# dmitrii-rudnev/selenite-lite

Hardware: AMD Instinct MI355X
Metric: Msamples/s complex I/Q through full RX chain (whole job) (higher is better)
Workload: dtype f32 in / out / accumulate; FIR multiplicands as exact f16 hi+lo pairs (~22 bits) on the matrix cores

## Files before the change

### include/selenite_rx.h

```cpp
#ifndef SELENITE_RX_H
#define SELENITE_RX_H

#include <stddef.h>
#include <stdint.h>

#ifdef __cplusplus
extern "C" {
#endif

#define SELENITE_RX_ABI_VERSION 2
#define SELENITE_RX_CONFIG_SIZE_V1 112u

#define SELENITE_RX_SUCCESS          0
#define SELENITE_RX_ARGUMENT_ERROR (-1)
#define SELENITE_RX_LENGTH_ERROR   (-2)
#define SELENITE_RX_NANINF         (-4)
#define SELENITE_RX_DEVICE_ERROR   (-7)

#define SELENITE_MODE_LSB 0x00
#define SELENITE_MODE_USB 0x01
#define SELENITE_MODE_CW  0x02
#define SELENITE_MODE_CWR 0x03
#define SELENITE_MODE_AM  0x04
#define SELENITE_MODE_FM  0x08
// ... 59 lines not shown

typedef struct selenite_rx_nr_state_view {
    float *coeffs;
    float *window;
    float *delay;
    float *energy;
    float *x0;
} selenite_rx_nr_state_view;

#define SELENITE_RX_OUT_MONO   0
#define SELENITE_RX_OUT_STEREO 1

typedef struct selenite_rx_out_config {
    uint32_t struct_size;
    uint32_t interp;
    uint32_t ni_taps;
    uint32_t frames;
    const float *coeffs;
} selenite_rx_out_config;

#define SELENITE_RX_WINDOW_HANN            0
#define SELENITE_RX_WINDOW_BLACKMAN_HARRIS 1

typedef struct selenite_rx_spec_config {
    uint32_t struct_size;
    uint32_t fft_len;
    uint32_t stride;
    uint32_t average;
    float alpha;
    const float *window;
} selenite_rx_spec_config;

typedef struct selenite_rx_spec_state_view {
    float *rows;
    float *pending;
    uint64_t *position;
} selenite_rx_spec_state_view;

typedef struct selenite_rx_instance selenite_rx_instance;


int  selenite_rx_init(selenite_rx_instance **S, const selenite_rx_config *cfg);
void selenite_rx_free(selenite_rx_instance *S);

int  selenite_rx_set_mode(selenite_rx_instance *S, uint8_t mode);

int  selenite_rx_status(const selenite_rx_instance *S);
const char *selenite_rx_error_string(const selenite_rx_instance *S);


void selenite_rx_process_f32(selenite_rx_instance *S, const float *pSrcIQ,
                             float *pDstAudio, uint32_t blockSize);

void *selenite_rx_host_alloc(size_t bytes);
void  selenite_rx_host_free(void *hptr);
int   selenite_rx_host_register(void *hptr, size_t bytes);
int   selenite_rx_host_unregister(void *hptr);

void selenite_rx_process_f32_device(selenite_rx_instance *S, const float *dSrcIQ,
                                    float *dDstAudio, uint32_t blockSize);

void selenite_rx_process_q15(selenite_rx_instance *S, const int16_t *pSrcIQ,
                             int16_t *pDstAudio, uint32_t blockSize);
void selenite_rx_process_q15_device(selenite_rx_instance *S, const int16_t *dSrcIQ,
                                    int16_t *dDstAudio, uint32_t blockSize);

void selenite_rx_global_phase1_device(selenite_rx_instance *S, const float *dSrcIQ,
                                      float *dDstAudio, float *dEnv, uint32_t blockSize);
void selenite_rx_global_phase2_device(selenite_rx_instance *S, float *dDstAudio,
                                      const float *dEnv, uint32_t blockSize);

int selenite_rx_global_process_f32_device(selenite_rx_instance *S, const float *dSrcIQ, float *dDstAudio,
                                          uint32_t blockSize, void *rccl_comm);


int selenite_rx_set_guard_ratio(selenite_rx_instance *S, float ratio);
int selenite_rx_guard_stats(selenite_rx_instance *S, uint64_t *guard_blocks, uint64_t *guard_channel_calls,
                            uint64_t *rerun_channel_calls);
int selenite_rx_guard_channels(selenite_rx_instance *S, uint32_t *per_channel);
int selenite_rx_auto_words(selenite_rx_instance *S, uint32_t *per_channel);
int selenite_rx_set_handover_repair(selenite_rx_instance *S, int on);
int selenite_rx_set_auto_launches(selenite_rx_instance *S, int launches);
int selenite_rx_auto_launches_last(const selenite_rx_instance *S);
int selenite_rx_guard_handover(selenite_rx_instance *S, uint64_t *handover_blocks);
int selenite_rx_guard_clear(selenite_rx_instance *S);


int  selenite_rx_set_stream(selenite_rx_instance *S, void *hip_stream);
int  selenite_rx_sync(selenite_rx_instance *S);

int  selenite_rx_get_state(selenite_rx_instance *S, const selenite_rx_state_view *dst);
int  selenite_rx_set_state(selenite_rx_instance *S, const selenite_rx_state_view *src);
int  selenite_rx_reset(selenite_rx_instance *S);


int  selenite_rx_set_nr(selenite_rx_instance *S, const selenite_rx_nr_config *nr);
int  selenite_rx_get_nr_state(selenite_rx_instance *S, const selenite_rx_nr_state_view *dst);
int  selenite_rx_set_nr_state(selenite_rx_instance *S, const selenite_rx_nr_state_view *src);


int      selenite_rx_set_out(selenite_rx_instance *S, const selenite_rx_out_config *out);
uint32_t selenite_rx_out_values(const selenite_rx_instance *S, uint32_t blockSize);
int      selenite_rx_get_out_state(selenite_rx_instance *S, float *interp_state);
int      selenite_rx_set_out_state(selenite_rx_instance *S, const float *interp_state);


int selenite_rx_set_spectrum(selenite_rx_instance *S, const selenite_rx_spec_config *sp);
int selenite_rx_get_spectrum(selenite_rx_instance *S, float *rows, uint64_t *frames);
const float *selenite_rx_spectrum_device(const selenite_rx_instance *S);
int selenite_rx_get_spectrum_state(selenite_rx_instance *S, const selenite_rx_spec_state_view *dst);
int selenite_rx_set_spectrum_state(selenite_rx_instance *S, const selenite_rx_spec_state_view *src);
int selenite_rx_spectrum_twiddles(float *tw, uint32_t fft_len);

void *selenite_rx_device_alloc(size_t bytes);
void  selenite_rx_device_free(void *dptr);
int   selenite_rx_memcpy_h2d(void *dptr, const void *hptr, size_t bytes);
int   selenite_rx_memcpy_d2h(void *hptr, const void *dptr, size_t bytes);
int   selenite_rx_device_count(void);
int   selenite_rx_set_device(int ordinal);


void selenite_rx_synth_iq_host(float *iq, uint32_t first_channel, uint32_t nch,
                               uint64_t first_sample, uint32_t nsamp, uint64_t seed);
int  selenite_rx_synth_iq_device(selenite_rx_instance *S, float *dIQ, uint32_t first_channel,
                                 uint32_t nch, uint64_t first_sample, uint32_t nsamp,
                                 uint64_t seed);

int  selenite_rx_time_process_device(selenite_rx_instance *S, const float *dSrcIQ,
                                     float *dDstAudio, uint32_t blockSize, uint32_t iters,
                                     float *ms_per_call);
int  selenite_rx_time_process_q15_device(selenite_rx_instance *S, const int16_t *dSrcIQ,
                                         int16_t *dDstAudio, uint32_t blockSize, uint32_t iters,
                                         float *ms_per_call);

int  selenite_rx_time_process_each_device(selenite_rx_instance *S, const void *dSrcIQ, void *dDstAudio, uint32_t blockSize,
                                          uint32_t iters, float *ms_each, int q15);
int  selenite_rx_time_streaming_roof_device(selenite_rx_instance *S, const void *dSrcIQ, void *dDstAudio, uint32_t blockSize,
                                            uint32_t iters, float *ms_each, int q15);
int  selenite_rx_time_pattern_roof_device(selenite_rx_instance *S, const void *dSrcIQ, void *dDstAudio, uint32_t blockSize,
                                          uint32_t iters, float *ms_each, int q15, uint32_t work);

#define SELENITE_RX_OPT_FORCE_GENERIC     0
#define SELENITE_RX_OPT_NO_SHARED_LO      1
#define SELENITE_RX_OPT_NO_PERIODIC_LO    2
#define SELENITE_RX_OPT_RERUN_GRID        3
#define SELENITE_RX_OPT_TX_FORCE_GENERIC  4
#define SELENITE_RX_OPT_CW_GRID           5
#define SELENITE_RX_OPT_COUNT             6
int      selenite_rx_set_plan_option(int option, uint32_t value);
uint32_t selenite_rx_get_plan_option(int option);
int  selenite_rx_device_pci_bus_id(int ordinal, char *buf, size_t len);

const char *selenite_rx_kernel_name(const selenite_rx_instance *S);
const char *selenite_rx_nco_path(const selenite_rx_instance *S);

uint64_t selenite_rx_algorithmic_bytes(const selenite_rx_config *cfg, uint32_t blockSize,
                                       uint64_t *read_bytes);


int selenite_rx_design_lowpass(float *coeffs, uint32_t num_taps, double cutoff);
int selenite_rx_design_hilbert(float *hilb, float *delay, uint32_t num_taps);
int selenite_rx_design_bandpass(float *coeffs, uint32_t n_stages, double f0, double q);

int selenite_rx_design_interp(float *coeffs, uint32_t ni_taps, uint32_t interp, double cutoff);

int selenite_rx_design_window(float *w, uint32_t n, int kind);
// ... 8 lines not shown
```

### selenite-lite_amd/csrc/rx_api.hip

```cpp
#include "rx_internal.h"

#include <cmath>
#include <cstddef>
#include <cstdio>
#include <cstdlib>
#include <cstring>
#include <algorithm>
#include <dlfcn.h>
#include <mutex>
#include <thread>

using namespace srx;

static thread_local std::string g_last_error = "";

static int fail(selenite_rx_instance *S, int code, const std::string &msg)
{
    g_last_error = msg;
    if (S) {
        if (S->status == SELENITE_RX_SUCCESS) S->status = code;
        S->err = msg;
    }
    return code;
}
#define HIPCHK(S, call)                                                                     \
    do {                                                                                    \
        hipError_t e_ = (call);                                                             \
        if (e_ != hipSuccess)                                                               \
            return fail((S), SELENITE_RX_DEVICE_ERROR,                                      \
                        std::string(#call) + ": " + hipGetErrorString(e_));                 \
    } while (0)

const float *srx::host_sin_table()
{
    static float table[513];
    static std::once_flag once;
    std::call_once(once, [] {
        for (int n = 0; n <= 512; ++n) {
            const double s = std::sin(2.0 * 3.14159265358979323846 * (double)n / 512.0);
            char buf[32];
            std::snprintf(buf, sizeof buf, "%.8f", s);
            table[n] = std::strtof(buf, nullptr);
        }
    });
    return table;
}

static bool mode_valid(uint8_t m, uint32_t nh_taps)
{
    if (m == SELENITE_MODE_FM) return nh_taps >= 2;
    return m == SELENITE_MODE_LSB || m == SELENITE_MODE_USB || m == SELENITE_MODE_CW ||
           m == SELENITE_MODE_CWR || m == SELENITE_MODE_AM || m == SELENITE_MODE_DIG ||
           m == SELENITE_MODE_PKT;
}

template <typename T>
static hipError_t dev_upload(T **d, const T *h, size_t n)
{
    *d = nullptr;
    if (n == 0) return hipSuccess;
    hipError_t e = hipMalloc((void **)d, n * sizeof(T));
    if (e != hipSuccess) return e;
    return hipMemcpy(*d, h, n * sizeof(T), hipMemcpyHostToDevice);
}
template <typename T>
static hipError_t dev_alloc(T **d, size_t n)
{
    *d = nullptr;
    if (n == 0) return hipSuccess;
    return hipMalloc((void **)d, n * sizeof(T));
}

static void classify_coeffs(selenite_rx_instance *S)
{
    const uint32_t nh = S->cfg.nh_taps;
    S->delay_is_impulse = false;
    S->hilb_odd_only = false;
    if (!nh) return;
    int ones = 0, idx = -1;
    bool rest_zero = true;
    for (uint32_t k = 0; k < nh; ++k) {
        const float v = S->h_delay[k];
        if (v == 1.0f) { ++ones; idx = (int)k; }
        else if (!(v == 0.0f && !std::signbit(v))) rest_zero = false;
    }
    if (ones == 1 && rest_zero) { S->delay_is_impulse = true; S->delay_index = idx; }
    if (nh % 2 == 1) {
        const int c = (int)(nh - 1) / 2;
        bool ok = true;
        for (uint32_t k = 0; k < nh && ok; ++k)
            if ((((int)k - c) & 1) == 0) {
                const float v = S->h_hilb[k];
                if (!(v == 0.0f && !std::signbit(v))) ok = false;
            }
        S->hilb_odd_only = ok;
    }
}

static void free_device(selenite_rx_instance *S)
{
    void *ptrs[] = { S->d_flags, S->d_guard_ch, S->d_rerun_flag, S->d_rerun_list, S->d_hist_ext, S->d_conv_in, S->d_dec_c, S->d_hilb_c, S->d_delay_c, S->d_biq_c, S->d_sintab, S->d_step, S->d_phase,
                     S->d_dec_state, S->d_fir_state, S->d_biq_state, S->d_gain, S->d_scratch, S->d_env, S->d_env_part,
                     S->d_io_in, S->d_io_out, S->d_lo, S->pipe.d_in[0], S->pipe.d_in[1], S->pipe.d_out[0], S->pipe.d_out[1],
                     S->d_nr_coeffs, S->d_nr_window, S->d_nr_delay, S->d_nr_energy, S->d_nr_x0,
                     S->d_out_coeffs, S->d_out_state, S->d_out_audio,
                     S->d_spec_tw, S->d_spec_window, S->d_spec_rows, S->d_spec_pending };
    for (void *p : ptrs)
        if (p) (void)hipFree(p);
    if (S->h_rerun_seen) (void)hipHostFree(S->h_rerun_seen);
    S->h_rerun_seen = nullptr;
    for (int i = 0; i < 2; ++i) {
        if (S->pipe.h_in[i]) (void)hipHostFree(S->pipe.h_in[i]);
        if (S->pipe.h_out[i]) (void)hipHostFree(S->pipe.h_out[i]);
        if (S->pipe.ev_in[i]) (void)hipEventDestroy(S->pipe.ev_in[i]);
        if (S->pipe.ev_done[i]) (void)hipEventDestroy(S->pipe.ev_done[i]);
        if (S->pipe.ev_out[i]) (void)hipEventDestroy(S->pipe.ev_out[i]);
    }
    if (S->pipe.h2d) (void)hipStreamDestroy(S->pipe.h2d);
    if (S->pipe.d2h) (void)hipStreamDestroy(S->pipe.d2h);
    free_fused(S->plan);
    if (S->own_stream) (void)hipStreamDestroy(S->own_stream);
}

static int nr_init_state(selenite_rx_instance *S)
{
    if (S->nr_kind == SELENITE_RX_NR_OFF) return SELENITE_RX_SUCCESS;
    const size_t C = S->cfg.channels, N = S->nr_taps, D = S->nr_delay;
    std::vector<float> w(C * N);
    for (size_t c = 0; c < C; ++c) std::memcpy(&w[c * N], S->h_nr_init.data(), N * sizeof(float));
    HIPCHK(S, hipMemcpyAsync(S->d_nr_coeffs, w.data(), C * N * sizeof(float), hipMemcpyHostToDevice, S->stream));
    HIPCHK(S, hipMemsetAsync(S->d_nr_window, 0, C * (N - 1) * sizeof(float), S->stream));
    HIPCHK(S, hipMemsetAsync(S->d_nr_delay, 0, C * D * sizeof(float), S->stream));
    HIPCHK(S, hipMemsetAsync(S->d_nr_energy, 0, C * sizeof(float), S->stream));
    HIPCHK(S, hipMemsetAsync(S->d_nr_x0, 0, C * sizeof(float), S->stream));
    HIPCHK(S, hipStreamSynchronize(S->stream));
    return SELENITE_RX_SUCCESS;
}

static int out_init_state(selenite_rx_instance *S)
{
    if (!S->out_on || S->out_taps / S->out_interp < 2) return SELENITE_RX_SUCCESS;
    const size_t n = (size_t)S->cfg.channels * (S->out_taps / S->out_interp - 1);
    HIPCHK(S, hipMemsetAsync(S->d_out_state, 0, n * sizeof(float), S->stream));
    HIPCHK(S, hipStreamSynchronize(S->stream));
    return SELENITE_RX_SUCCESS;
}

static int spec_init_state(selenite_rx_instance *S)
{
    if (!S->spec_len) return SELENITE_RX_SUCCESS;
    const size_t n = (size_t)S->cfg.channels * S->spec_len;
    HIPCHK(S, hipMemsetAsync(S->d_spec_rows, 0, n * sizeof(float), S->stream));
    HIPCHK(S, hipMemsetAsync(S->d_spec_pending, 0, 2 * n * sizeof(float), S->stream));
    HIPCHK(S, hipStreamSynchronize(S->stream));
    S->spec_pos = 0;
    return SELENITE_RX_SUCCESS;
}

static int reset_state(selenite_rx_instance *S)
{
    const selenite_rx_config &g = S->cfg;
    const size_t C = g.channels;
    if (g.nd_taps > 1) HIPCHK(S, hipMemsetAsync(S->d_dec_state, 0, C * 2 * (g.nd_taps - 1) * sizeof(float), S->stream));
    if (g.nh_taps > 1) HIPCHK(S, hipMemsetAsync(S->d_fir_state, 0, C * 2 * (g.nh_taps - 1) * sizeof(float), S->stream));
    if (g.n_biquad) HIPCHK(S, hipMemsetAsync(S->d_biq_state, 0, C * 4 * g.n_biquad * sizeof(float), S->stream));
    HIPCHK(S, hipMemsetAsync(S->d_phase, 0, C * sizeof(uint32_t), S->stream));
    HIPCHK(S, hipMemsetAsync(S->d_flags, 0, kFlagWords * sizeof(uint32_t), S->stream));
    HIPCHK(S, hipMemsetAsync(S->d_guard_ch, 0, 3 * C * sizeof(uint32_t), S->stream));
    if (S->d_rerun_flag) HIPCHK(S, hipMemsetAsync(S->d_rerun_flag, 0, C * sizeof(uint32_t), S->stream));
    if (S->d_rerun_list) HIPCHK(S, hipMemsetAsync(S->d_rerun_list, 0, 2 * sizeof(uint32_t), S->stream));
    S->rerun_par = 0;
    std::vector<float> gi(C, g.agc_gain_init);
    HIPCHK(S, hipMemcpyAsync(S->d_gain, gi.data(), C * sizeof(float), hipMemcpyHostToDevice, S->stream));
    HIPCHK(S, hipStreamSynchronize(S->stream));
    S->phase_uniform = true;
    S->phase_host = 0;
    if (int rc = nr_init_state(S)) return rc;
    if (int rc = out_init_state(S)) return rc;
    return spec_init_state(S);
}

static int check_device_flags(selenite_rx_instance *S)
{
    uint32_t f = 0;
// ... 51 lines not shown
            return fail(nullptr, SELENITE_RX_ARGUMENT_ERROR, "selenite_rx_init: q15_rounding is 0 or 1");
    } else {
        return fail(nullptr, SELENITE_RX_ARGUMENT_ERROR, "selenite_rx_init: struct_size matches neither this header's selenite_rx_config nor version 1's");
    }
    own.struct_size = (uint32_t)sizeof(selenite_rx_config);
    const selenite_rx_config *cfg = &own;
    if (cfg->channels == 0 || cfg->block == 0 || cfg->decim == 0)
        return fail(nullptr, SELENITE_RX_ARGUMENT_ERROR, "selenite_rx_init: channels, block, decim must be non-zero");
    if (!mode_valid(cfg->mode, cfg->nh_taps))
        return fail(nullptr, SELENITE_RX_ARGUMENT_ERROR, "selenite_rx_init: unsupported mode (FM needs the FIR pair's delay lines: nh_taps >= 2)");
    if (cfg->arith != SELENITE_ARITH_CMSIS && cfg->arith != SELENITE_ARITH_FMA && cfg->arith != SELENITE_ARITH_SPLIT16 &&
        cfg->arith != SELENITE_ARITH_AUTO)
        return fail(nullptr, SELENITE_RX_ARGUMENT_ERROR, "selenite_rx_init: bad arith");
    if (cfg->nd_taps == 0 && cfg->decim != 1)
        return fail(nullptr, SELENITE_RX_ARGUMENT_ERROR, "selenite_rx_init: decim > 1 needs a decimator (nd_taps)");
    if (cfg->nd_taps && !cfg->dec_coeffs)
        return fail(nullptr, SELENITE_RX_ARGUMENT_ERROR, "selenite_rx_init: dec_coeffs is NULL");
    if (cfg->nh_taps && (!cfg->hilb_coeffs || !cfg->delay_coeffs))
        return fail(nullptr, SELENITE_RX_ARGUMENT_ERROR, "selenite_rx_init: hilb_coeffs / delay_coeffs is NULL");
    if (cfg->n_biquad && !cfg->biquad_coeffs)
        return fail(nullptr, SELENITE_RX_ARGUMENT_ERROR, "selenite_rx_init: biquad_coeffs is NULL");
    if (cfg->nd_taps > 65535 || cfg->nh_taps > 65535 || cfg->decim > 255)
        return fail(nullptr, SELENITE_RX_ARGUMENT_ERROR, "selenite_rx_init: taps > 65535 or decim > 255");
    if (cfg->block % cfg->decim != 0)
        return fail(nullptr, SELENITE_RX_LENGTH_ERROR, "selenite_rx_init: block is not a multiple of decim");

    int ndev = 0;
    if (hipGetDeviceCount(&ndev) != hipSuccess || ndev <= 0)
        return fail(nullptr, SELENITE_RX_DEVICE_ERROR,
                    "selenite_rx_init: no HIP device (this library has no CPU fallback)");

    selenite_rx_instance *S = new selenite_rx_instance();
    S->cfg = *cfg;
    const size_t C = cfg->channels;
    if (cfg->nd_taps) S->h_dec.assign(cfg->dec_coeffs, cfg->dec_coeffs + cfg->nd_taps);
    if (cfg->nh_taps) {
        S->h_hilb.assign(cfg->hilb_coeffs, cfg->hilb_coeffs + cfg->nh_taps);
        S->h_delay.assign(cfg->delay_coeffs, cfg->delay_coeffs + cfg->nh_taps);
    }
    if (cfg->n_biquad) S->h_biq.assign(cfg->biquad_coeffs, cfg->biquad_coeffs + 5 * cfg->n_biquad);
    S->h_step.resize(C);
    for (size_t c = 0; c < C; ++c) S->h_step[c] = cfg->nco_step ? cfg->nco_step[c] : cfg->nco_step_all;
    S->cfg.dec_coeffs = S->h_dec.data(); S->cfg.hilb_coeffs = S->h_hilb.data();
    S->cfg.delay_coeffs = S->h_delay.data(); S->cfg.biquad_coeffs = S->h_biq.data();
    S->cfg.nco_step = S->h_step.data();
    S->steps_uniform = true;
    for (size_t c = 1; c < C; ++c) S->steps_uniform = S->steps_uniform && S->h_step[c] == S->h_step[0];
    S->steps_grid256 = true;
    for (size_t c = 0; c < C; ++c) S->steps_grid256 = S->steps_grid256 && (S->h_step[c] & 0x00FFFFFFu) == 0;
    S->force_generic = plan_option(SELENITE_RX_OPT_FORCE_GENERIC) ? 1 : 0;
    S->no_shared_lo = plan_option(SELENITE_RX_OPT_NO_SHARED_LO) ? 1 : 0;
    S->no_periodic_lo = plan_option(SELENITE_RX_OPT_NO_PERIODIC_LO) ? 1 : 0;

#define INITCHK(call)                                                                        \
    do {                                                                                     \
        hipError_t e_ = (call);                                                              \
        if (e_ != hipSuccess) {                                                              \
            int rc_ = fail(nullptr, SELENITE_RX_DEVICE_ERROR,                                \
                           std::string("selenite_rx_init: " #call ": ") + hipGetErrorString(e_)); \
            free_device(S);                                                                  \
            delete S;                                                                        \
            return rc_;                                                                      \
        }                                                                                    \
    } while (0)

    INITCHK(hipGetDevice(&S->device));
    INITCHK(hipStreamCreateWithFlags(&S->own_stream, hipStreamNonBlocking));
    S->stream = S->own_stream;
    INITCHK(dev_upload(&S->d_dec_c, S->h_dec.data(), S->h_dec.size()));
    INITCHK(dev_upload(&S->d_hilb_c, S->h_hilb.data(), S->h_hilb.size()));
    INITCHK(dev_upload(&S->d_delay_c, S->h_delay.data(), S->h_delay.size()));
    INITCHK(dev_upload(&S->d_biq_c, S->h_biq.data(), S->h_biq.size()));
    INITCHK(dev_upload(&S->d_sintab, host_sin_table(), (size_t)513));
    INITCHK(dev_upload(&S->d_step, S->h_step.data(), C));
    INITCHK(dev_alloc(&S->d_phase, C));
    INITCHK(dev_alloc(&S->d_dec_state, cfg->nd_taps > 1 ? C * 2 * (cfg->nd_taps - 1) : 0));
    INITCHK(dev_alloc(&S->d_fir_state, cfg->nh_taps > 1 ? C * 2 * (cfg->nh_taps - 1) : 0));
    INITCHK(dev_alloc(&S->d_biq_state, C * 4 * cfg->n_biquad));
    INITCHK(dev_alloc(&S->d_gain, C));
    INITCHK(dev_alloc(&S->d_flags, (size_t)kFlagWords));
    INITCHK(dev_alloc(&S->d_guard_ch, 3 * C));
    INITCHK(dev_alloc(&S->d_rerun_flag, cfg->arith == SELENITE_ARITH_AUTO ? C : 0));
    INITCHK(dev_alloc(&S->d_rerun_list, cfg->arith == SELENITE_ARITH_AUTO ? C + 2 : 0));
    if (cfg->arith == SELENITE_ARITH_AUTO) {
        INITCHK(hipHostMalloc(reinterpret_cast<void **>(&S->h_rerun_seen), sizeof(uint32_t), hipHostMallocMapped));
        *S->h_rerun_seen = 0u;
    }
    if (cfg->arith == SELENITE_ARITH_AUTO && cfg->nd_taps >= 2 && cfg->nh_taps >= 2 &&
        split16_template_nd((int)cfg->nd_taps, (int)cfg->decim, (int)cfg->nh_taps) > 0 && !diag_env("SELENITE_RX_NO_HIST_EXT")) {
        S->ext_len = cfg->decim * ((cfg->nh_taps - 1u + 3u) & ~3u);
    }
#undef INITCHK
    classify_coeffs(S);
    if (plan_fused(S->cfg, S->delay_is_impulse, S->delay_index, S->hilb_odd_only, S->plan) != hipSuccess) {
        int rc_ = fail(nullptr, SELENITE_RX_DEVICE_ERROR, "selenite_rx_init: building fused-kernel tables failed");
        free_device(S);
        delete S;
        return rc_;
    }
    int rc = reset_state(S);
    if (rc != SELENITE_RX_SUCCESS) { free_device(S); delete S; return rc; }
    *out = S;
    return SELENITE_RX_SUCCESS;
}

extern "C" void selenite_rx_free(selenite_rx_instance *S)
{
    if (!S) return;
    (void)hipSetDevice(S->device);
    if (S->stream) (void)hipStreamSynchronize(S->stream);
    free_device(S);
    delete S;
}

extern "C" int selenite_rx_set_mode(selenite_rx_instance *S, uint8_t mode)
{
    if (!S) return fail(nullptr, SELENITE_RX_ARGUMENT_ERROR, "selenite_rx_set_mode: S is NULL");
    if (!mode_valid(mode, S->cfg.nh_taps)) {
        g_last_error = "selenite_rx_set_mode: unsupported mode";
        return SELENITE_RX_ARGUMENT_ERROR;
    }
    S->cfg.mode = mode;
    HIPCHK(S, plan_fused(S->cfg, S->delay_is_impulse, S->delay_index, S->hilb_odd_only, S->plan));
    return SELENITE_RX_SUCCESS;
}

extern "C" int selenite_rx_status(const selenite_rx_instance *S) { return S ? S->status : SELENITE_RX_ARGUMENT_ERROR; }
extern "C" const char *selenite_rx_error_string(const selenite_rx_instance *S)
{
    return S ? S->err.c_str() : g_last_error.c_str();
}
extern "C" const char *selenite_rx_kernel_name(const selenite_rx_instance *S)
{
    if (!S) return "";
    if (S->force_generic) return "generic";
    if (S->plan.kind != 0) return S->plan.name;
    if (cw_fused_ok(S->cfg, S->cfg.block)) {
        static thread_local std::string name;
        name = "k_cw_fused<" + std::to_string(S->cfg.n_biquad) + "," + std::to_string(S->cfg.block) + ">";
        return name.c_str();
    }
    return "generic";
}

static bool periodic_lo(const selenite_rx_instance *S)
{
    const selenite_rx_config &g = S->cfg;
    if (!(g.nco_enable && S->steps_uniform && (S->h_step[0] & 0x00FFFFFFu) == 0 && !S->no_periodic_lo)) return false;
    if ((g.arith == SELENITE_ARITH_SPLIT16 || g.arith == SELENITE_ARITH_AUTO) && S->plan.d_btab16 && g.nd_taps)
        return 256u % (g.block / g.decim) == 0 && ssb_split16_periodic_lo(split16_template_nd((int)g.nd_taps, (int)g.decim, (int)g.nh_taps), (int)g.decim, (int)g.nh_taps);
    if (g.arith == SELENITE_ARITH_AUTO) return false;
    return g.arith != SELENITE_ARITH_CMSIS && S->plan.use_mfma && g.nd_taps && g.decim == 4;
}

static bool periodic_lo_per_channel(const selenite_rx_instance *S)
{
    const selenite_rx_config &g = S->cfg;
    if (!(g.nco_enable && S->steps_grid256 && !S->no_periodic_lo && S->plan.kind != 0)) return false;
    if (256u % (g.block / g.decim) != 0) return false;
    const bool split = (g.arith == SELENITE_ARITH_SPLIT16 || g.arith == SELENITE_ARITH_AUTO) && S->plan.d_btab16;
    if (split && g.nd_taps) return ssb_split16_periodic_lo(split16_template_nd((int)g.nd_taps, (int)g.decim, (int)g.nh_taps), (int)g.decim, (int)g.nh_taps);
    if (split) return false;
    const bool exact = g.arith == SELENITE_ARITH_CMSIS || g.arith == SELENITE_ARITH_AUTO;
    return exact || !(S->plan.use_mfma && g.decim == 4);
}

// ... 9 lines not shown
    }
    return periodic_lo(S) ? "shared LO, period 256 samples, held in registers" : "shared LO table per call";
}

extern "C" int selenite_rx_set_stream(selenite_rx_instance *S, void *hip_stream)
{
    if (!S) return SELENITE_RX_ARGUMENT_ERROR;
    hipStream_t next = hip_stream ? (hipStream_t)hip_stream : S->own_stream;
    if (next != S->stream) {
        HIPCHK(S, hipSetDevice(S->device));
        HIPCHK(S, hipStreamSynchronize(S->stream));
        S->stream = next;
    }
    return SELENITE_RX_SUCCESS;
}

extern "C" int selenite_rx_sync(selenite_rx_instance *S)
{
    if (!S) return SELENITE_RX_ARGUMENT_ERROR;
    HIPCHK(S, hipStreamSynchronize(S->stream));
    return check_device_flags(S);
}

extern "C" int selenite_rx_set_guard_ratio(selenite_rx_instance *S, float ratio)
{
    if (!S || !(ratio >= 0.0f)) return SELENITE_RX_ARGUMENT_ERROR;
    S->guard_ratio = ratio;
    return SELENITE_RX_SUCCESS;
}

extern "C" int selenite_rx_guard_stats(selenite_rx_instance *S, uint64_t *guard_blocks, uint64_t *guard_channel_calls,
                                       uint64_t *rerun_channel_calls)
{
    if (!S) return SELENITE_RX_ARGUMENT_ERROR;
    HIPCHK(S, hipSetDevice(S->device));
    HIPCHK(S, hipStreamSynchronize(S->stream));
    const size_t C = S->cfg.channels;
    std::vector<uint32_t> w(2 * C);
    HIPCHK(S, hipMemcpy(w.data(), S->d_guard_ch, 2 * C * sizeof(uint32_t), hipMemcpyDeviceToHost));
    uint64_t blocks = 0, calls = 0;
    for (size_t c = 0; c < C; ++c) { blocks += w[c]; calls += w[C + c]; }
    if (guard_blocks) *guard_blocks = blocks;
    if (guard_channel_calls) *guard_channel_calls = calls;
    if (rerun_channel_calls) *rerun_channel_calls = S->cfg.arith == SELENITE_ARITH_AUTO ? calls : 0;
    return SELENITE_RX_SUCCESS;
}

extern "C" int selenite_rx_guard_channels(selenite_rx_instance *S, uint32_t *per_channel)
{
    if (!S || !per_channel) return SELENITE_RX_ARGUMENT_ERROR;
    HIPCHK(S, hipSetDevice(S->device));
    HIPCHK(S, hipStreamSynchronize(S->stream));
    HIPCHK(S, hipMemcpy(per_channel, S->d_guard_ch, (size_t)S->cfg.channels * sizeof(uint32_t), hipMemcpyDeviceToHost));
    return SELENITE_RX_SUCCESS;
}

extern "C" int selenite_rx_auto_words(selenite_rx_instance *S, uint32_t *per_channel)
{
    if (!S || !per_channel) return SELENITE_RX_ARGUMENT_ERROR;
    HIPCHK(S, hipSetDevice(S->device));
    HIPCHK(S, hipStreamSynchronize(S->stream));
    if (!S->d_rerun_flag) { std::memset(per_channel, 0, (size_t)S->cfg.channels * sizeof(uint32_t)); return SELENITE_RX_SUCCESS; }
    HIPCHK(S, hipMemcpy(per_channel, S->d_rerun_flag, (size_t)S->cfg.channels * sizeof(uint32_t), hipMemcpyDeviceToHost));
    return SELENITE_RX_SUCCESS;
}

extern "C" int selenite_rx_guard_clear(selenite_rx_instance *S)
{
    if (!S) return SELENITE_RX_ARGUMENT_ERROR;
    HIPCHK(S, hipSetDevice(S->device));
    HIPCHK(S, hipMemsetAsync(S->d_guard_ch, 0, 3 * (size_t)S->cfg.channels * sizeof(uint32_t), S->stream));
    return SELENITE_RX_SUCCESS;
}

extern "C" int selenite_rx_set_auto_launches(selenite_rx_instance *S, int launches)
{
    if (!S || !(launches == 1 || launches == 3)) return SELENITE_RX_ARGUMENT_ERROR;
    S->auto_launches = launches;
    return SELENITE_RX_SUCCESS;
}

extern "C" int selenite_rx_auto_launches_last(const selenite_rx_instance *S)
{
    return S ? (int)S->auto_form_last : 0;
}

extern "C" int selenite_rx_set_handover_repair(selenite_rx_instance *S, int on)
{
    if (!S) return SELENITE_RX_ARGUMENT_ERROR;
    S->handover_repair = on != 0;
    if (!S->handover_repair && S->d_hist_ext) {
        HIPCHK(S, hipSetDevice(S->device));
        HIPCHK(S, hipStreamSynchronize(S->stream));
        const size_t C = S->cfg.channels;
        std::vector<uint32_t> w(C);
        HIPCHK(S, hipMemcpy(w.data(), S->d_rerun_flag, C * sizeof(uint32_t), hipMemcpyDeviceToHost));
        for (size_t c = 0; c < C; ++c)
            if (((w[c] >> kProvShift) & kProvMask) == kProvSplitExt)
                w[c] = (w[c] & ~((kProvMask << kProvShift) | kExtQ15)) | (kProvSplit << kProvShift);
        HIPCHK(S, hipMemcpy(S->d_rerun_flag, w.data(), C * sizeof(uint32_t), hipMemcpyHostToDevice));
        HIPCHK(S, hipFree(S->d_hist_ext));
        S->d_hist_ext = nullptr;
    }
    return SELENITE_RX_SUCCESS;
}

static int ensure_hist_ext(selenite_rx_instance *S)
{
    if (S->d_hist_ext || !S->ext_len || !S->handover_repair || !S->d_rerun_flag) return SELENITE_RX_SUCCESS;
    const size_t n = 2 * (size_t)S->cfg.channels * S->ext_len;
    HIPCHK(S, hipMalloc((void **)&S->d_hist_ext, n * sizeof(float2)));
    HIPCHK(S, hipMemsetAsync(S->d_hist_ext, 0, n * sizeof(float2), S->stream));
    return SELENITE_RX_SUCCESS;
}

extern "C" int selenite_rx_guard_handover(selenite_rx_instance *S, uint64_t *handover_blocks)
{
    if (!S || !handover_blocks) return SELENITE_RX_ARGUMENT_ERROR;
    HIPCHK(S, hipSetDevice(S->device));
    HIPCHK(S, hipStreamSynchronize(S->stream));
    const size_t C = S->cfg.channels;
    std::vector<uint32_t> w(C);
    HIPCHK(S, hipMemcpy(w.data(), S->d_guard_ch + 2 * C, C * sizeof(uint32_t), hipMemcpyDeviceToHost));
    uint64_t n = 0;
    for (size_t c = 0; c < C; ++c) n += w[c];
    *handover_blocks = n;
    return SELENITE_RX_SUCCESS;
}

extern "C" int selenite_rx_reset(selenite_rx_instance *S)
{
    if (!S) return SELENITE_RX_ARGUMENT_ERROR;
    return reset_state(S);
}

static void nr_release(selenite_rx_instance *S)
{
    float **bufs[] = { &S->d_nr_coeffs, &S->d_nr_window, &S->d_nr_delay, &S->d_nr_energy, &S->d_nr_x0 };
    for (float **b : bufs) {
        if (*b) (void)hipFree(*b);
        *b = nullptr;
    }
    S->nr_kind = SELENITE_RX_NR_OFF;
    S->nr_taps = S->nr_delay = 0;
    S->nr_mu = 0.0f;
    S->h_nr_init.clear();
}

extern "C" int selenite_rx_set_nr(selenite_rx_instance *S, const selenite_rx_nr_config *nr)
{
    if (!S) return fail(nullptr, SELENITE_RX_ARGUMENT_ERROR, "selenite_rx_set_nr: S is NULL");
    if (nr && nr->struct_size != sizeof(selenite_rx_nr_config)) {
        g_last_error = "selenite_rx_set_nr: struct_size is not sizeof(selenite_rx_nr_config)";
        return SELENITE_RX_ARGUMENT_ERROR;
    }
    if (nr && nr->kind != SELENITE_RX_NR_OFF) {
        const uint32_t N = nr->num_taps;
        const char *bad = nullptr;
        if (nr->kind != SELENITE_RX_NR_DENOISE && nr->kind != SELENITE_RX_NR_NOTCH) bad = "kind is not a SELENITE_RX_NR_* value";
        else if (N != 8 && N != 16 && N != 32 && N != 64) bad = "num_taps is not 8, 16, 32 or 64";
        else if (nr->delay < 1 || nr->delay > 64) bad = "delay is not 1 .. 64";
        else if (!(nr->mu > 0.0f && nr->mu < 2.0f)) bad = "mu is not finite in (0, 2)";
        else if (nr->coeffs_init)
            for (uint32_t k = 0; k < N && !bad; ++k)
                if (!std::isfinite(nr->coeffs_init[k])) bad = "coeffs_init holds a non-finite weight";
        if (bad) {
            g_last_error = std::string("selenite_rx_set_nr: ") + bad;
// ... 259 lines not shown
    q.coeffs = S->d_nr_coeffs; q.window = S->d_nr_window; q.delay_line = S->d_nr_delay; q.energy = S->d_nr_energy; q.x0 = S->d_nr_x0;
    q.flags = p.flags;
    if (S->sub_count) {
        const size_t c0 = S->sub_first;
        q.coeffs += c0 * S->nr_taps; q.window += c0 * (S->nr_taps - 1); q.delay_line += c0 * S->nr_delay;
        q.energy += c0; q.x0 += c0;
    }
    return q;
}

static int ensure(selenite_rx_instance *S, void **buf, size_t *cap, size_t need)
{
    if (*cap >= need) return SELENITE_RX_SUCCESS;
    if (*buf) { HIPCHK(S, hipStreamSynchronize(S->stream)); HIPCHK(S, hipFree(*buf)); *buf = nullptr; *cap = 0; }
    HIPCHK(S, hipMalloc(buf, need));
    *cap = need;
    return SELENITE_RX_SUCCESS;
}

static bool block_size_ok(selenite_rx_instance *S, uint32_t block_size, const char *who)
{
    if (block_size == 0 || block_size % S->cfg.block != 0) {
        fail(S, SELENITE_RX_LENGTH_ERROR, std::string(who) + ": blockSize is not a non-zero multiple of cfg.block");
        return false;
    }
    return true;
}

enum Phase { kAll, kPhase1, kPhase2 };

static int run_part(selenite_rx_instance *S, const void *src, bool src_q15, void *dst, bool dst_q15,
                    uint32_t block_size, Phase phase, float *ext_env, uint32_t in_stride, uint32_t out_stride)
{
    const selenite_rx_config &g = S->cfg;
    HIPCHK(S, hipSetDevice(S->device));
    if (phase != kPhase2 && S->plan.kind != 0 && S->plan.d_btab16 && !S->force_generic)
        if (int rc = ensure_hist_ext(S)) return rc;
    RxParams p = make_params(S, block_size);
    p.in_stride = in_stride; p.out_stride = out_stride;
    if (front_generic_lds_bytes(p) > 64 * 1024 && (S->force_generic || S->plan.kind == 0))
        return fail(S, SELENITE_RX_LENGTH_ERROR, "filter lengths exceed the LDS budget of the generic kernel");
    const int arith = (int)g.arith;
    const int garith = arith == SELENITE_ARITH_AUTO ? SELENITE_ARITH_CMSIS : arith;
    const bool global = g.agc_enable && g.agc_global;
    const bool cw = mode_is_cw(g.mode) && g.n_biquad;
    const bool nr = phase != kPhase2 && S->nr_kind != SELENITE_RX_NR_OFF;
    hipStream_t st = S->stream;

    const uint32_t phase_now = S->phase_host;
    auto commit_phase = [&]() { if (phase != kPhase2 && g.nco_enable) S->phase_host = phase_now + block_size * S->h_step[0]; };

    const bool fusable = phase != kPhase2 && !S->force_generic;
    const bool ssb_fused = fusable && S->plan.kind != 0;
    const bool cw_fused = fusable && cw_fused_ok(g, block_size) && cw_strides_ok(p.in_stride, p.out_stride);
    if ((global || nr) && src_q15 && (ssb_fused || cw_fused)) {
        const size_t nval = ((size_t)(p.channels - 1) * p.in_stride + block_size) * 2;
        if (nval % 8 == 0) {
            int rc = ensure(S, (void **)&S->d_conv_in, &S->conv_in_bytes, nval * sizeof(float));
            if (rc) return rc;
            HIPCHK(S, launch_q15_to_f32(static_cast<const int16_t *>(src), S->d_conv_in, nval, S->stream));
            src = S->d_conv_in;
            src_q15 = false;
        }
    }
    float *audio = (float *)dst;
    if (dst_q15 && (global || nr || !(ssb_fused || cw_fused))) {
        const size_t need = (size_t)g.channels * p.out_stride * sizeof(float);
        int rc = ensure(S, (void **)&S->d_scratch, &S->scratch_bytes, need);
        if (rc) return rc;
        audio = S->d_scratch;
    }
    if (phase != kPhase2 && S->d_rerun_flag && !ssb_fused) {
        uint32_t *words = S->d_rerun_flag + (S->sub_count ? S->sub_first : 0u);
        if (p.hist_ext) {
            RxParams ph = p;
            ph.chan_flags = words;
            HIPCHK(S, launch_hist_exact(ph, true, st));
        }
        HIPCHK(S, hipMemsetAsync(words, 0, p.channels * sizeof(uint32_t), st));
    }
    bool env_emitted = false;
    if (ssb_fused || cw_fused) {
        RxParams pf = p;
        if (g.nco_enable && S->steps_uniform && S->phase_uniform && !S->no_shared_lo) {
            const uint32_t lo_n = block_size < 256u ? 256u : block_size;
            if (!(S->lo_valid && S->lo_phase == phase_now && S->lo_step == S->h_step[0] && S->lo_n >= lo_n)) {
                S->lo_valid = false;
                int rc = ensure(S, (void **)&S->d_lo, &S->lo_bytes, (size_t)lo_n * sizeof(float2));
                if (rc) return rc;
                HIPCHK(S, launch_lo_table(S->d_lo, S->d_sintab, phase_now, S->h_step[0], lo_n, st));
                S->lo_valid = true; S->lo_phase = phase_now; S->lo_step = S->h_step[0]; S->lo_n = lo_n;
            }
            pf.nco = 2;
            pf.lo = S->d_lo;
            pf.lo_period = periodic_lo(S) ? 256u : 0u;
        } else if (ssb_fused && g.nco_enable && periodic_lo_per_channel(S)) {
            pf.lo_period = 256u;
        }
        if (arith == SELENITE_ARITH_AUTO && ssb_fused) {
            pf.rerun_flag = S->d_rerun_flag + (S->sub_count ? S->sub_first : 0u);
            pf.chan_list = S->d_rerun_list + 2;
            pf.chan_count = S->d_rerun_list;
            pf.rerun_par_host = &S->rerun_par;
            pf.rerun_seen = S->h_rerun_seen;
            pf.auto_inline = S->auto_launches == 1 ? 1u : 0u;
            pf.form_host = &S->auto_form_last;
        }
        void *fdst = dst;
        bool fq15 = dst_q15;
        if (global || nr) {
            pf.agc = 0; fdst = audio; fq15 = false;
            pf.out_cached = 1;
            if (!nr && ssb_fused && (arith == SELENITE_ARITH_SPLIT16 || arith == SELENITE_ARITH_AUTO) && S->plan.d_btab16 && g.nd_taps && g.decim == 4 && (g.block / g.decim) / 4 == 16 &&
                (block_size / g.decim) % 256 == 0 && g.nco_enable && g.mode != SELENITE_MODE_AM && g.mode != SELENITE_MODE_FM) {
                const size_t need = sizeof(float) * env_fold_scratch_floats(p.channels, block_size / g.block);
                int rc = ensure(S, (void **)&S->d_env_part, &S->env_part_cap, need);
                if (rc) return rc;
                pf.env_part = S->d_env_part;
                env_emitted = true;
            }
        }
        if (ssb_fused) HIPCHK(S, launch_fused(S->plan, pf, arith, src, src_q15, fdst, fq15, S->delay_index, st));
        else HIPCHK(S, launch_cw_fused(pf, src, src_q15, fdst, fq15, st));
        commit_phase();
        if (!global && !nr) return SELENITE_RX_SUCCESS;
    }

    if (phase != kPhase2 && !(ssb_fused || cw_fused)) {
        HIPCHK(S, launch_front_generic(p, garith, src, src_q15, audio, st));
        commit_phase();
        if (cw) HIPCHK(S, launch_biquad_generic(p, garith, audio, st));
    }
    if (nr) HIPCHK(S, launch_nlms(make_nr_params(S, p), S->nr_taps, audio, st));
    if (global) {
        float *env = ext_env;
        if (!env) {
            const size_t need = sizeof(float) * (block_size / g.block);
            int rc = ensure(S, (void **)&S->d_env, &S->env_cap, need);
            if (rc) return rc;
            env = S->d_env;
        }
        if (phase != kPhase2) {
            if (env_emitted) {
                HIPCHK(S, launch_env_fold(S->d_env_part, env, p.channels, block_size / g.block, st));
            } else {
                const size_t need = sizeof(float) * env_global_rows(p) * (block_size / g.block);
                int rc = ensure(S, (void **)&S->d_env_part, &S->env_part_cap, need);
                if (rc) return rc;
                HIPCHK(S, launch_env_global(p, audio, S->d_env_part, env, st));
            }
        }
        if (phase != kPhase1) HIPCHK(S, launch_agc_apply_global(p, garith, audio, env, dst, dst_q15, st));
    } else if (g.agc_enable || dst_q15) {
        HIPCHK(S, launch_agc_generic(p, garith, audio, dst, dst_q15, st));
    }
    return SELENITE_RX_SUCCESS;
}

static int run_chain_core(selenite_rx_instance *S, const void *src, bool src_q15, void *dst, bool dst_q15,
                          uint32_t block_size, Phase phase, float *ext_env)
{
    const selenite_rx_config &g = S->cfg;
    const uint32_t nout = block_size / g.decim;
    const bool global = g.agc_enable && g.agc_global;
    if (phase == kAll && !global && !S->force_generic && S->plan.kind != 0 && fused_tail_split(S->plan, g, block_size)) {
        const uint32_t unit = split16_pass_out(g.block, g.decim) * g.decim, bs1 = block_size / unit * unit;
        {
            int rc = run_part(S, src, src_q15, dst, dst_q15, bs1, kAll, nullptr, block_size, nout);
            if (rc) return rc;
            const size_t ein = src_q15 ? sizeof(int16_t) : sizeof(float), eout = dst_q15 ? sizeof(int16_t) : sizeof(float);
            const char *src2 = static_cast<const char *>(src) + (size_t)bs1 * 2 * ein;
            char *dst2 = static_cast<char *>(dst) + (size_t)(bs1 / g.decim) * eout;
            return run_part(S, src2, src_q15, dst2, dst_q15, block_size - bs1, kAll, nullptr, block_size, nout);
        }
    }
    return run_part(S, src, src_q15, dst, dst_q15, block_size, phase, ext_env, block_size, nout);
}

static int out_audio(selenite_rx_instance *S, uint32_t block_size, float **audio)
{
    const size_t nch = S->sub_count ? S->sub_count : S->cfg.channels;
    int rc = ensure(S, (void **)&S->d_out_audio, &S->out_audio_bytes, nch * (block_size / S->cfg.decim) * sizeof(float));
    *audio = S->d_out_audio;
    return rc;
}
static int out_finish(selenite_rx_instance *S, const float *audio, void *dst, bool dst_q15, uint32_t block_size)
{
    OutParams q{};
// ... 524 lines not shown
```

### selenite-lite_amd/csrc/rx_fused.hip

```cpp
#include "rx_fused_kernels.h"

#include <cmath>
#include <cstdio>
#include <cstdlib>

#pragma clang fp contract(off)

namespace srx {

template <int ND, int M, int NH>
struct GeoM {
    using G = Geo<ND, M, NH>;
    static constexpr int HS = G::HQ4 * M;
    static constexpr int XN = HS + G::T;
    static constexpr int XROWS = XN / 64;
    static constexpr int XLEN = 66 * XROWS;
    static constexpr int KTOT = ND + 4 * 15 + 1;
    static constexpr int KS = (KTOT + 3) / 4;
    static constexpr int oTab = 0;
    static constexpr int oX = 516;
    static constexpr int oD = oX + 2 * XLEN;
    static constexpr int total = oD + 2 * G::DLEN;
    __host__ __device__ static constexpr int phys(int f) { return f + 2 * (f >> 6); }
};
// ... 340 lines not shown
        if (NH > 0) {
            const int nds = split16_template_nd(ndr, M, NH);
            constexpr int MT = M == 8 ? 4 : M;
#define X(ND_, M_, NH_) if (nds == ND_ && MT == M_ && NH == NH_) return build_split16_table<ND_, M_, NH_>(g, plan);
            SRX_SPLIT16_SHAPES(X)
#undef X
        }
        return hipSuccess;
    }
    if constexpr (ND == 0 && M == 1 && NH > 0) {
        using GH = GeoH<NH>;
        float cmax = 0.0f;
        for (int k = 0; k < NH; ++k) cmax = std::fmax(cmax, std::fabs(g.hilb_coeffs[k]));
        int ex = 0;
        if (cmax > 0.0f) std::frexp(cmax, &ex);
        const int SC = 15 - ex;
        std::vector<_Float16> b16((size_t)GH::KS * 2 * 64 * 8, (_Float16)0.0f);
        for (int kk = 0; kk < GH::KS; ++kk)
            for (int l = 0; l < 64; ++l)
                for (int j = 0; j < 8; ++j) {
                    const int idx = 32 * kk + 8 * (l >> 4) + j - (l & 15);
                    float cv = 0.0f;
                    if (idx >= 0 && idx < NH) cv = std::ldexp(g.hilb_coeffs[idx], SC);
                    const _Float16 hi = (_Float16)cv;
                    const _Float16 lo = (_Float16)(cv - (float)hi);
                    b16[(((size_t)2 * kk + 0) * 64 + l) * 8 + j] = hi;
                    b16[(((size_t)2 * kk + 1) * 64 + l) * 8 + j] = lo;
                }
        hipError_t e = hipMalloc(&plan.d_btab16, b16.size() * sizeof(_Float16));
        if (e != hipSuccess) return e;
        e = hipMemcpy(plan.d_btab16, b16.data(), b16.size() * sizeof(_Float16), hipMemcpyHostToDevice);
        if (e != hipSuccess) return e;
        plan.split_sc = SC;
    }
    return hipSuccess;
}


template <int ND, int M, int NH, typename TIn, typename TOut>
static hipError_t launch_mfma(const RxParams &p, const FusedArgs &fa, const float *btab, const void *src, void *dst,
                              hipStream_t st)
{
    using GM = GeoM<ND, M, NH>;
    constexpr size_t lds = (size_t)kMfmaWaves * GM::total * sizeof(float);
    static_assert(lds <= 160 * 1024, "k_ssb_mfma LDS image");
    const uint32_t nco = (p.nco == 2 && p.lo_period == 256 && Geo<ND, M, NH>::T % 256 == 0) ? 3u : p.nco;
    auto k = fa.am ? (nco == 3 ? k_ssb_mfma<3, ND, M, NH, TIn, TOut, 1> : nco == 2 ? k_ssb_mfma<2, ND, M, NH, TIn, TOut, 1>
                         : (nco == 1 ? k_ssb_mfma<1, ND, M, NH, TIn, TOut, 1> : k_ssb_mfma<0, ND, M, NH, TIn, TOut, 1>))
                   : (nco == 3 ? k_ssb_mfma<3, ND, M, NH, TIn, TOut, 0> : nco == 2 ? k_ssb_mfma<2, ND, M, NH, TIn, TOut, 0>
                         : (nco == 1 ? k_ssb_mfma<1, ND, M, NH, TIn, TOut, 0> : k_ssb_mfma<0, ND, M, NH, TIn, TOut, 0>));
    hipError_t e = hipFuncSetAttribute(reinterpret_cast<const void *>(k), hipFuncAttributeMaxDynamicSharedMemorySize,
                                       (int)lds);
    if (e != hipSuccess) return e;
    static int resident = 0;
    if (resident == 0) {
        int per_cu = 0, dev = 0;
        hipDeviceProp_t prop;
        if (hipOccupancyMaxActiveBlocksPerMultiprocessor(&per_cu, k, 64 * kMfmaWaves, lds) == hipSuccess && per_cu > 0 &&
            hipGetDevice(&dev) == hipSuccess && hipGetDeviceProperties(&prop, dev) == hipSuccess)
            resident = per_cu * prop.multiProcessorCount;
        else
            resident = -1;
        if (const char *ge = diag_env("SELENITE_RX_MFMA_GRID")) resident = std::atoi(ge) > 0 ? std::atoi(ge) : -1;
    }
    uint32_t grid = p.channels / kMfmaWaves;
    if (resident > 0 && (uint32_t)resident < grid) grid = (uint32_t)resident;
    hipLaunchKernelGGL(k, dim3(grid), dim3(64 * kMfmaWaves), lds, st, p, fa, btab,
                       static_cast<const TIn *>(src), static_cast<TOut *>(dst));
    return hipGetLastError();
}

template <int ND, int M, int NH>
static hipError_t launch_shape(const RxParams &p, const FusedArgs &fa, const FusedPlan &plan, int arith,
                               const void *src, bool src_q15, void *dst, bool dst_q15, hipStream_t st)
{
    if (src_q15 != dst_q15) return hipErrorNotSupported;
    const bool auto_ = arith == SELENITE_ARITH_AUTO;
    const bool fm = fa.am == 2u;
    const bool split = (arith == SELENITE_ARITH_SPLIT16 || auto_) && !(fm && !(auto_ && ND > 0));
    auto rerun = [&]() -> hipError_t {
        RxParams p2 = p;
        p2.chan_flags = p.rerun_flag;
        p2.rerun_flag = nullptr;
        if (p.rerun_par_host) {
            const uint32_t par = *p.rerun_par_host & 1u;
            p2.chan_count = p.chan_count + par;
            p2.chan_count_next = p.chan_count + (par ^ 1u);
            *p.rerun_par_host = par ^ 1u;
        }
        if (hipError_t e = launch_hist_exact(p2, false, st); e != hipSuccess) return e;
        return launch_exact(ND, M, NH, src_q15, p2, fa, src, dst, st);
    };
    const bool whole = fa.pass_out == 256 && p.nout % 256 == 0;
    const int nds = ND > 0 ? split16_template_nd((int)p.nd, M, NH) : -1;
    const uint32_t kHS = nds > 0 ? (uint32_t)(((((nds - 1 + M - 1) / M) + 3) & ~3) * M) : 0u;
    FusedArgs fa16 = fa;
    if constexpr (M == 8) {
        fa16.pass_out = split16_pass_out(p.block, p.decim);
        static const uint32_t par = [] {
            const char *e = diag_env("SELENITE_RX_DEC2_PARITY");
            if (e && e[0] == '2' && e[1] == 0) { fprintf(stderr, "selenite_rx: SELENITE_RX_DEC2_PARITY=2 -- decimation by 8 keeps the ODD by-4 outputs (diagnostic, wrong audio)\n"); return 2u; }
            return 1u;
        }();
        fa16.dec2 = par;
    }
    const uint32_t tq = fa16.pass_out * M;
    const bool split_ok = split16_pass_ok(fa16.pass_out) && (p.block_size % tq == 0 || p.block_size % tq >= kHS || p.block_size < tq);
    const bool auto_ok = !auto_ || p.hist_ext == nullptr || p.block_size + 1u >= (uint32_t)(ND > 0 ? p.nd - 1 : 0) + p.ext_len;
    if constexpr (ND > 0 && (M == 4 || M == 2 || M == 8) && NH > 0) {
        if (split && plan.d_btab16 && split_ok && auto_ok) {
            if (auto_ && fa.am == 1u && p.rerun_flag) {
                RxParams p3 = p;
                p3.chan_flags = p.rerun_flag;
                p3.chan_list = nullptr; p3.chan_count_next = nullptr;
                if (hipError_t e = launch_hist_exact(p3, true, st); e != hipSuccess) return e;
            }
            if (auto_ && p.rerun_flag && p.form_host) *p.form_host = 3u;
            hipError_t e = launch_ssb_split16(nds, M == 8 ? 4 : M, NH, p, fa16, src, src_q15, dst, st);
            if (e == hipSuccess && auto_ && p.rerun_flag) e = rerun();
            return e;
        }
    }
    if constexpr (ND == 0 && M == 1 && NH > 0) {
        const bool hilb_ok = fa.pass_out != 0;
        if (split && plan.d_btab16 && hilb_ok) {
            FusedArgs fah = fa;
            const bool inl = auto_ && p.rerun_flag && p.auto_inline && !fa.am;
            fah.inl = inl ? 1u : 0u;
            if (auto_ && p.rerun_flag && p.form_host) *p.form_host = inl ? 1u : 3u;
            hipError_t e = launch_hilb_split16(NH, p, fah, src, src_q15, dst, st);
            if (e == hipSuccess && auto_ && p.rerun_flag && !inl) e = rerun();
            return e;
        }
    }
    if (auto_) {
        arith = SELENITE_ARITH_CMSIS;
        if (p.rerun_flag) {
            RxParams p3 = p;
            p3.chan_flags = p.rerun_flag;
            p3.chan_list = nullptr; p3.chan_count_next = nullptr;
            if (hipError_t e = launch_hist_exact(p3, true, st); e != hipSuccess) return e;
        }
    }
    if constexpr (ND > 0 && M == 4) {
        static_assert(kMfmaWaves == 1, "one channel per workgroup: any channel count launches (plan.name says k_ssb_mfma)");
        if (arith != SELENITE_ARITH_CMSIS && plan.use_mfma && whole) {
            if (src_q15) return launch_mfma<ND, M, NH, int16_t, int16_t>(p, fa, plan.d_btab, src, dst, st);
            return launch_mfma<ND, M, NH, float, float>(p, fa, plan.d_btab, src, dst, st);
        }
    }
    if (arith != SELENITE_ARITH_CMSIS) {
        if (src_q15) return launch_one<1, ND, M, NH, int16_t, int16_t>(p, fa, src, dst, st);
        return launch_one<1, ND, M, NH, float, float>(p, fa, src, dst, st);
    }
    return launch_exact(ND, M, NH, src_q15, p, fa, src, dst, st);
}


static bool fused_mode_ok(const selenite_rx_config &g)
{
    const uint32_t m = g.mode;
    const bool ssb = m == SELENITE_MODE_USB || m == SELENITE_MODE_LSB || m == SELENITE_MODE_DIG || m == SELENITE_MODE_PKT;
    const bool cw_plain = mode_is_cw(m) && g.n_biquad == 0;
    return ssb || cw_plain || m == SELENITE_MODE_AM || m == SELENITE_MODE_FM;
}

hipError_t plan_fused(const selenite_rx_config &g, bool delay_is_impulse, int delay_index, bool hilb_odd_only,
                      FusedPlan &plan)
{
    (void)delay_index;
    plan.kind = 0;
    plan.dense = false;
    plan.name = "generic";
    if (!fused_mode_ok(g) || !g.nh_taps) return hipSuccess;
    const uint32_t na = g.block / g.decim;
    if (na < 4 || na > 256 || na % 4 != 0) return hipSuccess;
    int kind = 0;
    const char *name = nullptr;
    if (delay_is_impulse && hilb_odd_only) {
#define X(ND_, M_, NH_, ID_) \
    if (shape_is<ND_, M_, NH_>(g)) { kind = ID_; name = "k_ssb_fused<" #ND_ "," #M_ "," #NH_ ">"; }
    SRX_SHAPES(X)
#undef X
    }
    if (!kind) {
        if (g.nh_taps > 127) return hipSuccess;
        int nds = -1;
#define X(ND_, M_, NH_, ID_) \
        if ((int)g.decim == M_ && ((int)g.nd_taps == 0 ? ND_ == 0 : (ND_ >= (int)g.nd_taps && (int)g.nd_taps >= 2)) && (nds < 0 || ND_ < nds)) { nds = ND_; kind = ID_; }
        SRX_DENSE_SHAPES(X)
#undef X
        if (!kind) return hipSuccess;
        if (!plan.tables_built) {
            hipError_t e = hipSuccess;
#define X(ND_, M_, NH_, ID_) if (kind == ID_) e = build_tables<ND_, M_, NH_>(g, plan, true);
            SRX_DENSE_SHAPES(X)
#undef X
            if (e != hipSuccess) return e;
            constexpr int NHT = 127, LEN = DenseTab<NHT>::LEN, FH = ((NHT - 1 + 3) & ~3) - (NHT - 1);
            std::vector<float> pt((size_t)2 * LEN, 0.0f);
            const int pad = NHT - (int)g.nh_taps;
            for (int k = 0; k < (int)g.nh_taps; ++k) {
                pt[(size_t)k + pad + FH + 3] = g.delay_coeffs[k];
                pt[(size_t)LEN + k + pad + FH + 3] = g.hilb_coeffs[k];
            }
            e = hipMalloc((void **)&plan.d_ptab, pt.size() * sizeof(float));
            if (e != hipSuccess) return e;
            e = hipMemcpy(plan.d_ptab, pt.data(), pt.size() * sizeof(float), hipMemcpyHostToDevice);
            if (e != hipSuccess) return e;
            plan.dense_t0 = (uint32_t)((pad + FH - 3) > 0 ? (pad + FH - 3) / 4 : 0);
            plan.tables_built = true;
        }
// ... 117 lines not shown
```

### selenite-lite_amd/csrc/rx_fused_kernels.h

```cpp
#pragma once
#include "rx_fused_common.h"
#include "rx_hist_exact.h"

#include <cmath>
#include <cstdio>
#include <cstdlib>

#pragma clang fp contract(off)

namespace srx {


template <int ARITH, int ND, int M, int NH>
__device__ __forceinline__ void decim_quad(const float *S, int lane, const float (&creg)[Geo<ND, M, NH>::NCR],
                                           v2f (&acc)[4])
{
    using G = Geo<ND, M, NH>;
    const float *base = S + 12 * lane;
#pragma unroll
    for (int o = 0; o < (G::HQ4 + 4) / 2; ++o) {
        float4 W[M];
#pragma unroll
        for (int p = 0; p < M; ++p)
            W[p] = lds_ld4f(base + p * G::PSF + 4 * (3 * (o >> 1) + (o & 1)));
// ... 149 lines not shown
            if (off < group) m = fmaxf(m, __shfl_xor(m, off, 64));
    } else {
        float mm = 0.0f;
        for (int j = 0; j < group; ++j) mm = fmaxf(mm, __shfl(m, ((lane / group) * group + j) & 63, 64));
        m = mm;
    }
    {
        const bool first = lane % gl == 0 && lane / gl < nvb;
        if (env_row && first) env_row[lane / gl] = m;
        if (gx) {
            gx->n += (uint32_t)__builtin_popcountll(__builtin_amdgcn_ballot_w64(first && m < gx->thr));
            gx->n2 += (uint32_t)__builtin_popcountll(__builtin_amdgcn_ballot_w64(first && m < gx->thr2));
        }
    }
    if (p.agc) {
        float g = gain, mine = gain;
        if constexpr (GROUP > 0) {
            const int myblk = lane / GROUP;
            float dsr[64 / GROUP];
            const float mine_d = agc_desired(p.agcp, m);
#pragma unroll
            for (int b = 0; b < 64 / GROUP; ++b)
                dsr[b] = __int_as_float(__builtin_amdgcn_readlane(__float_as_int(mine_d), b * GROUP));
#pragma unroll
            for (int b = 0; b < 64 / GROUP; ++b) {
                const float gn = agc_step(p.agcp, g, dsr[b]);
                g = b < nvb ? gn : g;
                mine = (b == myblk) ? g : mine;
            }
        } else {
            const int myblk = lane / group;
            const int nblk = min(64 / group, nvb);
            for (int b = 0; b < nblk; ++b) {
                const float env = __shfl(m, b * group, 64);
                g = agc_update<0>(p.agcp, g, env);
                if (b == myblk) mine = g;
            }
        }
        gain = g;
#pragma unroll
        for (int r = 0; r < 4; ++r) au[r] = au[r] * mine;
    }
    const bool live = lane < nvb * (GROUP ? GROUP : group);
    {
        const float z = __builtin_fmaf(au[3], 0.0f, __builtin_fmaf(au[2], 0.0f, __builtin_fmaf(au[1], 0.0f, au[0] * 0.0f)));
        nonfinite = nonfinite || (live && z != z);
    }
    const size_t o = out_index + 4 * lane;
    if (live) {
        if constexpr (sizeof(TOut) == 4) {
            v4f *at = reinterpret_cast<v4f *>(reinterpret_cast<float *>(dst) + o);
            const v4f av = { au[0], au[1], au[2], au[3] };
            if (p.out_cached) *at = av;
            else asm volatile("global_store_dwordx4 %0, %1, off nt\n\ts_nop 1" :: "v"(at), "v"(av) : "memory");
        } else {
            typedef uint32_t w2v __attribute__((ext_vector_type(2)));
            uint32_t w0, w1;
            float4_to_q15(au[0], au[1], au[2], au[3], p.q15_round, w0, w1);
            __builtin_nontemporal_store(w2v{ w0, w1 }, reinterpret_cast<w2v *>(reinterpret_cast<int16_t *>(dst) + o));
        }
    }
}

struct FusedInl { uint32_t c, word; };
template <int ARITH, int ND, int M, int NH, typename TIn, typename TOut, int DENSE, bool INL>
__device__ __forceinline__ void ssb_fused_body(RxParams p, FusedArgs fa, const TIn *__restrict__ src, TOut *__restrict__ dst, FusedInl inl)
{
    using G = Geo<ND, M, NH>;
    const uint32_t NCO = fa.nco;
    constexpr int AM = 2;
    const int ndr = ND > 0 ? (int)p.nd : 0, Fr = ND > 0 ? G::HQ4 * M + 1 - ndr : 0;
    const int hhr = NH > 0 ? (int)p.nh - 1 : 0, FHr = G::HH4 - hhr;
    using R = BRaw<TIn>;
    static_assert(ND == 0 ? M == 1 : (M == 2 || M == 4 || M == 8), "fused kernel: no decimator, or decimate by 2, 4 or 8");
    extern __shared__ __attribute__((aligned(16))) float lds[];
    const int lane = threadIdx.x;
    const uint32_t pq = fa.pass_out, tq = pq * M;
    float *tab = lds + G::oTab;
    float *S = lds + G::oS;
    float *D = lds + G::oD;
    float *dI = D, *dQ = D + G::DLEN;
    constexpr int NLD = G::T / 128;
    bool nonfinite = false;
    uint32_t li = INL ? 0u : blockIdx.x;
    const uint32_t ln = INL ? 1u : (p.chan_flags ? *p.chan_count : 0u);
    if (!INL && p.chan_flags && p.rerun_seen && blockIdx.x == 0 && lane == 0) __hip_atomic_store(p.rerun_seen, ln, __ATOMIC_RELAXED, __HIP_MEMORY_SCOPE_SYSTEM);
    if (p.chan_flags && li >= ln) return;
    if (NCO == 1u || NCO == 4u)
        for (int i = lane; i < 513; i += kWave) tab[i] = p.sintab[i];
    float creg[G::NCR > 0 ? G::NCR : 1];
    if constexpr (ND > 0) {
#pragma unroll
        for (int v = 0; v < G::NCR; ++v) creg[v] = fa.cq[64 * v + lane];
    }
    float hreg[(NH + 63) / 64 ? (NH + 63) / 64 : 1];
#pragma unroll
    for (int v = 0; v < (NH + 63) / 64; ++v) hreg[v] = (DENSE == 0 && 64 * v + lane < NH) ? p.hilb_c[64 * v + lane] : 0.0f;
    if constexpr (DENSE != 0) {
        float *pt = lds + G::total;
        for (int i = lane; i < 2 * DenseTab<NH>::LEN; i += kWave) pt[i] = fa.ptab[i];
        fa.ptab_lds = pt;
    }
    auto in_rsrc = [&](uint32_t ch, bool valid) { return make_rsrc(src + (size_t)ch * p.in_stride * 2, valid ? p.block_size * (R::kBytes / 2) : 0u); };
    uint32_t c_cur = INL ? inl.c : blockIdx.x;
    if (!INL && p.chan_flags) c_cur = li < ln ? p.chan_list[li] : 0u;
    typename R::type raw[NLD];
    {
        const __amdgpu_buffer_rsrc_t rs0 = in_rsrc(c_cur, !p.chan_flags || li < ln);
#pragma unroll
        for (int i = 0; i < NLD; ++i) raw[i] = R::load(rs0, lane * R::kBytes + i * 64 * R::kBytes, 0);
    }
  for (;;) {
    const uint32_t c = c_cur;
    uint32_t c_nxt = 0u;
    bool has_nxt = false;
    if (p.chan_flags) {
        if (li >= ln) break;
        li += INL ? 1u : gridDim.x;
        has_nxt = li < ln;
        c_nxt = has_nxt ? p.chan_list[li] : 0u;
    }

    const size_t out_base = (size_t)c * p.out_stride;
    const uint32_t npass = (p.nout + pq - 1) / pq;
    const bool rerun_pass = p.chan_flags != nullptr;
    const uint32_t word_in = INL ? inl.word : (rerun_pass ? p.chan_flags[c] : 0u);
    const bool held_in = (word_in & kFlagHold) != 0u;
    GuardEx gx{ 0.0f, 0.0f, 0u, 0u };
    float hmax = 0.0f;
    const __amdgpu_buffer_rsrc_t rs_in = in_rsrc(c, true);
    const __amdgpu_buffer_rsrc_t rs_next = in_rsrc(c_nxt, has_nxt);
    const __amdgpu_buffer_rsrc_t rs_lo = make_rsrc(p.lo, NCO == 2u ? p.block_size * 8u : 0u);

    if constexpr (ND > 0) {
        batched_fill<2 * M * G::HQ4>(lane, p.dec_state + (size_t)c * 2 * (ndr - 1),
            [&](int i) {
                const int rail = i / (M * G::HQ4), sidx = i % (M * G::HQ4) - Fr;
                return sidx >= 0 ? rail * (ndr - 1) + sidx : -1;
            },
            [&](int i, float v) {
                const int rail = i / (M * G::HQ4), rem = i % (M * G::HQ4);
                S[(rem % M) * G::PSF + G::elem(rem / M) + rail] = v;
                hmax = fmaxf(hmax, fabsf(v));
            });
    }
    if constexpr (NH > 0) {
        batched_fill<2 * G::HH4>(lane, p.fir_state + (size_t)c * 2 * hhr,
            [&](int i) {
                const int rail = i / G::HH4, sidx = i % G::HH4 - FHr;
                return sidx >= 0 ? rail * hhr + sidx : -1;
            },
            [&](int i, float v) { D[(i / G::HH4) * G::DLEN + i % G::HH4] = v; if (ND == 0) hmax = fmaxf(hmax, fabsf(v)); });
    }
    float pm_prev = __uint_as_float(wave_umax_bits(hmax));
    const uint32_t ph0 = NCO ? p.phase[c] : 0u;
    const uint32_t step = NCO ? p.step[c] : 0u;
    float gain = p.agc ? p.gain[c] : 1.0f;
    const int group = (int)fa.group;
    wave_lds_sync();
    lo_v2f lo_per[4] = { { 1.0f, 0.0f }, { 1.0f, 0.0f }, { 1.0f, 0.0f }, { 1.0f, 0.0f } };
    if (NCO == 4u) {
        const uint32_t pe = ph0 + 2u * lane * step;
        nco_lo_pair(tab, pe, pe + step, lo_per[0], lo_per[1]);
        nco_lo_pair(tab, pe + 128u * step, pe + 129u * step, lo_per[2], lo_per[3]);
    }

    for (uint32_t pass = 0; pass < npass; ++pass) {
        const uint32_t n0 = pass * tq;
        const uint32_t cur = (pass + 1 == npass) ? p.nout - pass * pq : pq;
        float mx = 0.0f;
        constexpr int CH = NLD < 8 ? NLD : 8;
        static_assert(NLD % CH == 0, "whole chunks");
        const bool mixing = NCO != 0u;
#pragma unroll
        for (int ch = 0; ch < NLD / CH; ++ch) {
        lo_v2f la[CH], lb[CH];
        if (NCO == 2u) {
            u4v lo4[CH];
#pragma unroll
            for (int j = 0; j < CH; ++j)
                lo4[j] = __builtin_amdgcn_raw_buffer_load_b128(rs_lo, lane * 16 + (ch * CH + j) * 1024, (int)(n0 * 8u), 0);
            __builtin_amdgcn_sched_barrier(0);
#pragma unroll
            for (int j = 0; j < CH; ++j) {
                la[j] = lo_v2f{ __uint_as_float(lo4[j].x), __uint_as_float(lo4[j].y) };
                lb[j] = lo_v2f{ __uint_as_float(lo4[j].z), __uint_as_float(lo4[j].w) };
            }
        } else if (NCO == 1u) {
#pragma unroll
            for (int j = 0; j < CH; ++j) {
                const uint32_t pe = ph0 + (n0 + 128u * (ch * CH + j) + 2u * lane) * step;
                nco_lo_pair(tab, pe, pe + step, la[j], lb[j]);
            }
        } else {
#pragma unroll
            for (int j = 0; j < CH; ++j) { la[j] = lo_per[2 * (j & 1)]; lb[j] = lo_per[2 * (j & 1) + 1]; }
        }
        auto mix_scatter = [&](auto mixc) {
            constexpr bool MIX = decltype(mixc)::value;
#pragma unroll
        for (int j = 0; j < CH; ++j) {
            const int i = ch * CH + j;
            const uint32_t n = 128u * i + 2u * lane;
            float2 a, b;
            {
                v2f va, vb;
                R::unpack(raw[i], va, vb);
                a = make_float2(va.x, va.y); b = make_float2(vb.x, vb.y);
            }
            if constexpr (MIX) {
// ... 183 lines not shown
```

### selenite-lite_amd/csrc/rx_generic.hip

```cpp
#include "rx_internal.h"
#include "rx_hist_exact.h"

#include <type_traits>

#pragma clang fp contract(off)

namespace srx {

static __host__ __device__ inline uint32_t up4(uint32_t v) { return (v + 3u) & ~3u; }

typedef float v2f __attribute__((ext_vector_type(2)));

struct FrontLds {
    uint32_t tab, cd, chd, S, D, Hq, F, PL, total;
};
static __host__ __device__ inline FrontLds front_layout(uint32_t nd, uint32_t nh, uint32_t M, uint32_t P, bool nco)
{
    FrontLds L;
    const uint32_t Hh = nh ? nh - 1 : 0;
    L.Hq = nd ? (nd - 1 + M - 1) / M : 0;
    L.F = nd ? L.Hq * M - (nd - 1) : 0;
    L.PL = L.Hq + P;
    uint32_t o = 0;
    L.tab = o; o += nco ? 516u : 0u;
// ... 402 lines not shown
hipError_t launch_front_generic(const RxParams &p, int arith, const void *src, bool src_q15,
                                float *audio, hipStream_t st)
{
    if (arith != SELENITE_ARITH_CMSIS)
        return src_q15 ? front_launch<1, int16_t>(p, src, audio, st) : front_launch<1, float>(p, src, audio, st);
    return src_q15 ? front_launch<0, int16_t>(p, src, audio, st) : front_launch<0, float>(p, src, audio, st);
}

hipError_t launch_biquad_generic(const RxParams &p, int arith, float *audio, hipStream_t st)
{
    const dim3 grid((p.channels + 63) / 64), blk(64);
    if (arith != SELENITE_ARITH_CMSIS) hipLaunchKernelGGL(k_biquad_generic<1>, grid, blk, 0, st, p, audio);
    else hipLaunchKernelGGL(k_biquad_generic<0>, grid, blk, 0, st, p, audio);
    return hipGetLastError();
}

hipError_t launch_agc_generic(const RxParams &p, int arith, const float *audio, void *dst,
                              bool dst_q15, hipStream_t st)
{
    const dim3 grid(p.channels), blk(64);
    if (arith != SELENITE_ARITH_CMSIS) {
        if (dst_q15) hipLaunchKernelGGL((k_agc_generic<1, int16_t>), grid, blk, 0, st, p, audio, (int16_t *)dst);
        else hipLaunchKernelGGL((k_agc_generic<1, float>), grid, blk, 0, st, p, audio, (float *)dst);
    } else {
        if (dst_q15) hipLaunchKernelGGL((k_agc_generic<0, int16_t>), grid, blk, 0, st, p, audio, (int16_t *)dst);
        else hipLaunchKernelGGL((k_agc_generic<0, float>), grid, blk, 0, st, p, audio, (float *)dst);
    }
    return hipGetLastError();
}

constexpr uint32_t kEnvColsGrid = 256, kEnvColsThreads = 256;
__global__ __launch_bounds__(kEnvColsThreads) void k_env_cols(const float *part, float *out, size_t total)
{
    const size_t j = (size_t)blockIdx.x * kEnvColsThreads + threadIdx.x, n = (size_t)gridDim.x * kEnvColsThreads;
    float m = 0.0f;
    for (size_t i = j; i < total; i += n) m = fmaxf(m, part[i]);
    out[j] = m;
}

size_t env_fold_scratch_floats(uint32_t rows, uint32_t nblk)
{
    return (size_t)rows * nblk + (size_t)kEnvColsGrid * kEnvColsThreads;
}

hipError_t launch_env_fold(float *part, float *env, uint32_t rows, uint32_t nblk, hipStream_t st)
{
    const uint32_t n = kEnvColsGrid * kEnvColsThreads;
    if (rows > 4096 && n % nblk == 0) {
        float *cols = part + (size_t)rows * nblk;
        hipLaunchKernelGGL(k_env_cols, dim3(kEnvColsGrid), dim3(kEnvColsThreads), 0, st, part, cols, (size_t)rows * nblk);
        hipLaunchKernelGGL(k_env_fold, dim3(nblk), dim3(kFoldThreads), 0, st, cols, env, n / nblk, nblk);
    } else {
        hipLaunchKernelGGL(k_env_fold, dim3(nblk), dim3(kFoldThreads), 0, st, part, env, rows, nblk);
    }
    return hipGetLastError();
}

uint32_t env_global_rows(const RxParams &p)
{
    const uint32_t grid = (p.channels + kEnvWaves - 1) / kEnvWaves;
    return (grid < kEnvMaxGrid ? grid : kEnvMaxGrid) * kEnvWaves;
}

hipError_t launch_env_global(const RxParams &p, const float *audio, float *part, float *env, hipStream_t st)
{
    const uint32_t rows = env_global_rows(p), nblk = p.block_size / p.block;
    hipLaunchKernelGGL(k_env_global, dim3(rows / kEnvWaves), dim3(64 * kEnvWaves), 0, st, p, audio, part);
    hipLaunchKernelGGL(k_env_fold, dim3(nblk), dim3(kFoldThreads), 0, st, part, env, rows, nblk);
    return hipGetLastError();
}

__global__ __launch_bounds__(256) void k_q15_to_f32(const int16_t *__restrict__ src, float *__restrict__ dst, size_t n8)
{
    typedef short s8v __attribute__((ext_vector_type(8)));
    for (size_t i = (size_t)blockIdx.x * blockDim.x + threadIdx.x; i < n8; i += (size_t)gridDim.x * blockDim.x) {
        const s8v v = __builtin_nontemporal_load(reinterpret_cast<const s8v *>(src) + i);
        v4f a = { q15_to_float(v[0]), q15_to_float(v[1]), q15_to_float(v[2]), q15_to_float(v[3]) };
        v4f b = { q15_to_float(v[4]), q15_to_float(v[5]), q15_to_float(v[6]), q15_to_float(v[7]) };
        __builtin_nontemporal_store(a, reinterpret_cast<v4f *>(dst) + 2 * i);
        __builtin_nontemporal_store(b, reinterpret_cast<v4f *>(dst) + 2 * i + 1);
    }
}

hipError_t launch_hist_exact(const RxParams &p, bool all, hipStream_t st)
{
    if (!p.chan_flags) return hipSuccess;
    static const bool off = diag_env("SELENITE_RX_NO_HIST_EXACT") != nullptr;
    const bool repair = p.hist_ext && p.nd >= 2 && p.nh >= 2 && !off;
    if (!repair && !p.chan_list) return hipSuccess;
    const uint32_t nwin = (p.channels + 63u) / 64u;
    const size_t lds = repair ? 2 * (size_t)(p.ext_len + p.nd - 1u) * sizeof(float) : 0;
    hipLaunchKernelGGL(k_hist_exact, dim3(nwin < 1024u ? nwin : 1024u), dim3(64), lds, st, p, all ? 1u : 0u, repair ? 1u : 0u);
    return hipGetLastError();
}

hipError_t launch_q15_to_f32(const int16_t *src, float *dst, size_t n, hipStream_t st)
{
    if (n % 8 != 0) return hipErrorInvalidValue;
    const size_t n8 = n / 8;
    const unsigned grid = (unsigned)((n8 + 255) / 256 < 16384 ? (n8 + 255) / 256 : 16384);
    hipLaunchKernelGGL(k_q15_to_f32, dim3(grid ? grid : 1), dim3(256), 0, st, src, dst, n8);
    return hipGetLastError();
}

hipError_t launch_agc_apply_global(const RxParams &p, int arith, const float *audio, const float *env,
                                   void *dst, bool dst_q15, hipStream_t st)
{
    const uint32_t na = p.block / p.decim;
    if (!dst_q15 && na >= 4 && 256u % na == 0 && p.nout % 256u == 0 && p.out_stride % 4u == 0) {
        if (arith != SELENITE_ARITH_CMSIS) hipLaunchKernelGGL(k_agc_apply_global_rows<1>, dim3(p.channels), dim3(64), 0, st, p, audio, env, (float *)dst);
        else hipLaunchKernelGGL(k_agc_apply_global_rows<0>, dim3(p.channels), dim3(64), 0, st, p, audio, env, (float *)dst);
        return hipGetLastError();
    }
    const uint32_t cpw = (na % 4 == 0 && na / 4 < 64) ? 64 / (na / 4) : 1;
    const dim3 grid((p.channels + cpw - 1) / cpw), blk(64);
    if (arith != SELENITE_ARITH_CMSIS) {
        if (dst_q15) hipLaunchKernelGGL((k_agc_apply_global<1, int16_t>), grid, blk, 0, st, p, audio, env, (int16_t *)dst);
        else hipLaunchKernelGGL((k_agc_apply_global<1, float>), grid, blk, 0, st, p, audio, env, (float *)dst);
    } else {
        if (dst_q15) hipLaunchKernelGGL((k_agc_apply_global<0, int16_t>), grid, blk, 0, st, p, audio, env, (int16_t *)dst);
        else hipLaunchKernelGGL((k_agc_apply_global<0, float>), grid, blk, 0, st, p, audio, env, (float *)dst);
    }
    return hipGetLastError();
}

}
```

### selenite-lite_amd/csrc/rx_internal.h

```cpp
#pragma once
#include <hip/hip_runtime.h>
#include <stdint.h>
#include <string>
#include <vector>

#include "../../include/selenite_rx.h"
#include "rx_device.h"
#include "rx_diag.h"

namespace srx {

struct RxParams {
    uint32_t channels;
    uint32_t block;
    uint32_t decim;
    uint32_t nd;
    uint32_t nh;
    uint32_t nbiq;
    uint32_t mode;
    uint32_t nco;
    uint32_t agc;
    uint32_t block_size;
    uint32_t nout;
    uint32_t in_stride;
    uint32_t out_stride;
    uint32_t pass_out;
    uint32_t q15_round;
    uint32_t out_cached;
    const float *dec_c, *hilb_c, *delay_c, *biq_c, *sintab;
    const float2 *lo;
    uint32_t lo_period;
    const uint32_t *step;
    uint32_t *phase;
    float *dec_state;
    float *fir_state;
    float *biq_state;
    float *gain;
    float *env_part;
    uint32_t *flags;
    float guard_ratio;
    uint32_t *guard_ch;
    uint32_t *guard_calls;
    uint32_t *guard_hand;
    uint32_t *rerun_flag;
    float2 *hist_ext;
    uint32_t ext_len;
    size_t ext_buf_stride;
    uint32_t *chan_flags;
    uint32_t *chan_list;
    uint32_t *chan_count;
    uint32_t *chan_count_next;
    uint32_t *rerun_par_host;
    uint32_t auto_inline;
    uint32_t *form_host;
    uint32_t *rerun_seen;
    AgcParams agcp;
};

enum { kFlagNanInf = 0, kFlagWords = 4 };
enum : uint32_t { kFlagRerun = 1u, kProvShift = 1u, kProvMask = 3u, kProvExact = 0u, kProvSplitExt = 1u, kProvSplit = 2u, kExtBufShift = 3u,
                  kExtQ15 = 16u,
                  kFlagHold = 32u,
                  kFlagClean1 = 64u,
                  kLvlMask = 0xFFFFFF00u };

__host__ __device__ inline bool mode_is_cw(uint32_t m) { return m == SELENITE_MODE_CW || m == SELENITE_MODE_CWR; }
__host__ __device__ inline bool mode_is_upper(uint32_t m)
{
    return m == SELENITE_MODE_USB || m == SELENITE_MODE_DIG || m == SELENITE_MODE_CW;
}

hipError_t launch_front_generic(const RxParams &p, int arith, const void *src, bool src_q15,
                                float *audio, hipStream_t st);
size_t front_generic_lds_bytes(const RxParams &p);
hipError_t launch_q15_to_f32(const int16_t *src, float *dst, size_t n, hipStream_t st);
hipError_t launch_hist_exact(const RxParams &p, bool all, hipStream_t st);
hipError_t launch_biquad_generic(const RxParams &p, int arith, float *audio, hipStream_t st);
hipError_t launch_agc_generic(const RxParams &p, int arith, const float *audio, void *dst,
                              bool dst_q15, hipStream_t st);
uint32_t env_global_rows(const RxParams &p);
hipError_t launch_env_global(const RxParams &p, const float *audio, float *part, float *env, hipStream_t st);
size_t env_fold_scratch_floats(uint32_t rows, uint32_t nblk);
hipError_t launch_env_fold(float *part, float *env, uint32_t rows, uint32_t nblk, hipStream_t st);
hipError_t launch_agc_apply_global(const RxParams &p, int arith, const float *audio, const float *env,
                                   void *dst, bool dst_q15, hipStream_t st);

struct NrParams {
    uint32_t channels;
    uint32_t nout;
    uint32_t stride;
    uint32_t delay;
    uint32_t notch;
    float mu;
    float *coeffs;
    float *window;
    float *delay_line;
    float *energy;
    float *x0;
    uint32_t *flags;
};
hipError_t launch_nlms(const NrParams &q, uint32_t num_taps, float *audio, hipStream_t st);

struct OutParams {
    uint32_t channels;
    uint32_t nout;
    uint32_t stride;
    uint32_t phase_len;
    uint32_t q15_round;
    uint32_t vec;
    const float *coeffs;
    float *state;
    uint32_t *flags;
};
inline uint32_t out_sample_bytes(bool stereo, bool q15) { return (q15 ? 2u : 4u) * (stereo ? 2u : 1u); }
hipError_t launch_out(const OutParams &q, uint32_t interp, bool stereo, bool dst_q15, const float *audio, void *dst, hipStream_t st);
hipError_t launch_q15_to_f32_any(const int16_t *src, float *dst, size_t n, hipStream_t st);

struct SpecParams {
    uint32_t channels;
    uint32_t block_size;
    uint32_t in_stride;
    uint32_t off;
    uint32_t first;
    uint32_t stride;
    uint32_t average;
    float alpha;
    const float *tw;
    const float *window;
    float *rows;
    float *pending;
};
hipError_t launch_spectrum(const SpecParams &q, uint32_t fft_len, const void *src, bool src_q15, hipStream_t st);
void spec_twiddles(float *tw, uint32_t n);

struct FusedPlan {
    int kind = 0;
    const char *name = "generic";
    std::string name_buf;
    float *d_cq = nullptr;
    float *d_btab = nullptr;
    void *d_btab16 = nullptr;
    float split_post = 1.0f;
    int split_sc = 0;
    bool use_mfma = false;
    bool dense = false;
    float *d_ptab = nullptr;
    uint32_t dense_t0 = 0;
    bool dense_delay_impulse = false;
    bool tables_built = false;
};
hipError_t plan_fused(const selenite_rx_config &cfg, bool delay_is_impulse, int delay_index,
                      bool hilb_odd_only, FusedPlan &plan);
void free_fused(FusedPlan &plan);
inline bool split16_pass_ok(uint32_t pass_out) { return pass_out != 0 && pass_out <= 256u && pass_out % 16u == 0; }
inline uint32_t split16_pass_out(uint32_t block, uint32_t decim)
{
    const uint32_t na = decim ? block / decim : 0u;
    return na ? (decim == 8u ? 128u : 256u) / na * na : 0u;
}
bool fused_tail_split(const FusedPlan &plan, const selenite_rx_config &cfg, uint32_t block_size);
hipError_t launch_fused(const FusedPlan &plan, const RxParams &p, int arith, const void *src,
                        bool src_q15, void *dst, bool dst_q15, int delay_index, hipStream_t st);

int fused_template_nd(int nd, int m, int nh);
int split16_template_nd(int nd, int m, int nh);
bool ssb_split16_periodic_lo(int nd, int m, int nh);
bool ssb_split16_has_shape(int nd, int m, int nh);

bool cw_fused_ok(const selenite_rx_config &cfg, uint32_t block_size);
bool cw_strides_ok(uint64_t in_stride, uint64_t out_stride);
hipError_t launch_cw_roof(const RxParams &p, const void *src, bool q15, void *dst, float4 *state, uint32_t work, hipStream_t st);
hipError_t launch_cw_fused(const RxParams &p, const void *src, bool src_q15, void *dst, bool dst_q15, hipStream_t st);

hipError_t launch_lo_table(float2 *lo, const float *sintab, uint32_t phase0, uint32_t step, uint32_t nsamp,
                           hipStream_t st);

hipError_t launch_synth(float *dIQ, const float *sintab, uint32_t first_channel, uint32_t nch,
                        uint64_t first_sample, uint32_t nsamp, uint64_t seed, hipStream_t st);
void synth_host(float *iq, const float *sintab, uint32_t first_channel, uint32_t nch,
                uint64_t first_sample, uint32_t nsamp, uint64_t seed);

hipError_t launch_stream_roof(const void *in, void *out, float *state, uint32_t channels, uint32_t in_bytes, uint32_t out_bytes,
                              uint32_t state_words, hipStream_t st);

const float *host_sin_table();

}

struct selenite_rx_instance {
    selenite_rx_config cfg;
    std::vector<float> h_dec, h_hilb, h_delay, h_biq;
    std::vector<uint32_t> h_step;
    int device = 0;
    hipStream_t own_stream = nullptr, stream = nullptr;
    float *d_dec_c = nullptr, *d_hilb_c = nullptr, *d_delay_c = nullptr, *d_biq_c = nullptr, *d_sintab = nullptr;
    uint32_t *d_step = nullptr, *d_phase = nullptr;
    float *d_dec_state = nullptr, *d_fir_state = nullptr, *d_biq_state = nullptr, *d_gain = nullptr;
    uint32_t *d_flags = nullptr;
    uint32_t *d_guard_ch = nullptr;
    uint32_t *d_rerun_flag = nullptr;
    uint32_t *d_rerun_list = nullptr;
    uint32_t rerun_par = 0;
    uint32_t *h_rerun_seen = nullptr;
    int auto_launches = 1;
    uint32_t auto_form_last = 0;
    float2 *d_hist_ext = nullptr;
    uint32_t ext_len = 0;
    bool handover_repair = true;
    float guard_ratio = 0.25f;
    bool steps_grid256 = false;
    float *d_scratch = nullptr;  size_t scratch_bytes = 0;
    float *d_conv_in = nullptr;  size_t conv_in_bytes = 0;
    float *d_env = nullptr;      size_t env_cap = 0;
    float *d_env_part = nullptr; size_t env_part_cap = 0;
    void *d_io_in = nullptr;     size_t io_in_bytes = 0;
    void *d_io_out = nullptr;    size_t io_out_bytes = 0;
    struct HostPipe {
        hipStream_t h2d = nullptr, d2h = nullptr;
        hipEvent_t ev_in[2] = { nullptr, nullptr }, ev_done[2] = { nullptr, nullptr }, ev_out[2] = { nullptr, nullptr };
        void *d_in[2] = { nullptr, nullptr }, *d_out[2] = { nullptr, nullptr };
        void *h_in[2] = { nullptr, nullptr }, *h_out[2] = { nullptr, nullptr };
        size_t d_in_bytes = 0, d_out_bytes = 0, h_in_bytes = 0, h_out_bytes = 0;
    } pipe;
    uint32_t sub_first = 0, sub_count = 0;
    float2 *d_lo = nullptr;      size_t lo_bytes = 0;
    bool lo_valid = false; uint32_t lo_phase = 0, lo_step = 0, lo_n = 0;
    bool steps_uniform = false;
    bool phase_uniform = true;
    uint32_t phase_host = 0;
    bool delay_is_impulse = false; int delay_index = 0; bool hilb_odd_only = false;
    srx::FusedPlan plan;
    int no_shared_lo = 0;
    int no_periodic_lo = 0;
    int force_generic = 0;
    uint32_t nr_kind = SELENITE_RX_NR_OFF, nr_taps = 0, nr_delay = 0;
    float nr_mu = 0.0f;
    std::vector<float> h_nr_init;
    float *d_nr_coeffs = nullptr, *d_nr_window = nullptr, *d_nr_delay = nullptr, *d_nr_energy = nullptr, *d_nr_x0 = nullptr;
    bool out_on = false;
    uint32_t out_interp = 1, out_taps = 0, out_frames = SELENITE_RX_OUT_MONO;
    float *d_out_coeffs = nullptr, *d_out_state = nullptr;
    float *d_out_audio = nullptr; size_t out_audio_bytes = 0;
    uint32_t spec_len = 0, spec_stride = 1, spec_average = 0;
    float spec_alpha = 1.0f;
    uint64_t spec_pos = 0;
    float *d_spec_tw = nullptr, *d_spec_window = nullptr;
    float *d_spec_rows = nullptr, *d_spec_pending = nullptr;
    int status = SELENITE_RX_SUCCESS;
    std::string err;
};
```

### selenite-lite_amd/csrc/rx_split16_kernels.h

```cpp
#pragma once
#include "rx_fused_kernels.h"

#include <cstdlib>
#include <type_traits>

#pragma clang fp contract(off)

namespace srx {

__device__ __forceinline__ float st_ld(const float *p)
{
    return *p;
}
__device__ __forceinline__ void st_st(float *p, float v)
{
    *p = v;
}

__device__ __forceinline__ uint32_t sat_add_u32(uint32_t a, uint32_t b) { return a > 0xFFFFFFFFu - b ? 0xFFFFFFFFu : a + b; }

__device__ __forceinline__ float amax2(v2f x, float m) { return fmaxf(fmaxf(fabsf(x.x), fabsf(x.y)), m); }

__device__ __forceinline__ void lds_order()
{
// ... 43 lines not shown
        const uint32_t r0 = __builtin_amdgcn_readlane(__float_as_uint(m), 0), r1 = __builtin_amdgcn_readlane(__float_as_uint(m), 16);
        const uint32_t r2 = __builtin_amdgcn_readlane(__float_as_uint(m), 32), r3 = __builtin_amdgcn_readlane(__float_as_uint(m), 48);
        const float e0 = __uint_as_float(r0 > r1 ? r0 : r1), e1 = __uint_as_float(r2 > r3 ? r2 : r3);
        guard(lane < 32 ? e0 : e1);
        const float d = agc_desired(ap, lane < 32 ? e0 : e1);
        const float ds[2] = { __uint_as_float(__builtin_amdgcn_readlane(__float_as_uint(d), 0)),
                              __uint_as_float(__builtin_amdgcn_readlane(__float_as_uint(d), 32)) };
        const int myblk = lane >> 5;
#pragma unroll
        for (int b = 0; b < 2; ++b) {
            const float gn = agc_step(ap, g, ds[b]);
            g = b < nvb ? gn : g;
            mine = (b == myblk) ? g : mine;
        }
    } else if constexpr (GROUP == 64) {
        m = __uint_as_float(wave_umax_bits_dpp(m));
        guard(m);
        g = agc_step(ap, g, agc_desired(ap, m));
        mine = g;
    } else {
        if ((group & 15) == 0) {
            m = row16_fmax(m);
            const uint32_t r0 = __builtin_amdgcn_readlane(__float_as_uint(m), 0), r1 = __builtin_amdgcn_readlane(__float_as_uint(m), 16);
            const uint32_t r2 = __builtin_amdgcn_readlane(__float_as_uint(m), 32), r3 = __builtin_amdgcn_readlane(__float_as_uint(m), 48);
            const int rows = group >> 4;
            uint32_t e0 = r0, e1 = r1, e2 = r2, e3 = r3;
            if (rows == 2) { e0 = e1 = max(r0, r1); e2 = e3 = max(r2, r3); }
            else if (rows == 3) { e0 = e1 = e2 = max(max(r0, r1), r2); }
            else if (rows >= 4) { e0 = e1 = e2 = e3 = max(max(r0, r1), max(r2, r3)); }
            const int row = lane >> 4;
            m = __uint_as_float(row == 0 ? e0 : (row == 1 ? e1 : (row == 2 ? e2 : e3)));
        } else if (group == 8) {
            m = fmaxf(m, __uint_as_float((uint32_t)__builtin_amdgcn_update_dpp(0, (int)__float_as_uint(m), 0xB1, 0xf, 0xf, false)));
            m = fmaxf(m, __uint_as_float((uint32_t)__builtin_amdgcn_update_dpp(0, (int)__float_as_uint(m), 0x4E, 0xf, 0xf, false)));
            m = fmaxf(m, __uint_as_float((uint32_t)__builtin_amdgcn_update_dpp(0, (int)__float_as_uint(m), 0x141, 0xf, 0xf, false)));
        } else if ((group & (group - 1)) == 0) {
#pragma unroll
            for (int off = 1; off < 64; off <<= 1)
                if (off < group) m = fmaxf(m, __shfl_xor(m, off, 64));
        } else {
            const int seg_end = (lane / group + 1) * group;
            for (int off = 1; off < group; off <<= 1) {
                const float v = __shfl_down(m, off, 64);
                m = lane + off < seg_end ? fmaxf(m, v) : m;
            }
        }
        guard(m);
        const float d = agc_desired(ap, m);
        const int nblk = min(64 / group, nvb), myblk = lane / group;
        for (int b = 0; b < nblk; ++b) {
            g = agc_step(ap, g, __uint_as_float(__builtin_amdgcn_readlane(__float_as_uint(d), b * group)));
            if (b == myblk) mine = g;
        }
    }
    gain = agc_on ? g : gain;
    mine = agc_on ? mine : 1.0f;
#pragma unroll
    for (int r = 0; r < 4; ++r) au[r] = au[r] * mine;
}

template <int NCO, int ND, int M, int NH, typename TIn, typename TOut, int AM, int GROUP, int FLAVOUR = 0>
__global__ __launch_bounds__(64, 2) void k_ssb_split16(RxParams p, FusedArgs fa, const TIn *__restrict__ src,
                                                       TOut *__restrict__ dst)
{
    constexpr int ENV = FLAVOUR == 1 ? 1 : 0;
    constexpr bool DEC2 = FLAVOUR == 2;
    static_assert(!DEC2 || GROUP == 0, "decimation by 2 M: run-time geometry only");
    using G = Geo<ND, M, NH>;
    using GS = GeoS<NCO, ND, M, NH>;
    using R = BRaw<TIn>;
    using W = BOut<TOut>;
    static_assert(ND > 0 && (M == 4 || M == 2) && NH > 0 && G::T % 128 == 0 && GS::HS % 128 == 0, "split16 decimator: /4 or /2, + Hilbert");
    extern __shared__ __attribute__((aligned(16))) float lds[];
    const int lane = threadIdx.x;
    const bool fm = AM != 0 && fa.am == 2u;
    const bool keeps = AM == 0 || fm;
    uint64_t ch_mask = 0ull;
    uint32_t ch_lo = blockIdx.x;
    auto ch_scan = [&](uint32_t &w, bool &mine) {
        const uint64_t ci = (uint64_t)ch_lo + (uint64_t)lane * gridDim.x;
        mine = ci < (uint64_t)p.channels;
        w = p.rerun_flag != nullptr ? p.rerun_flag[mine ? ci : 0] : 0u;
    };
    auto ch_take = [&](uint32_t w, bool mine) {
        ch_mask = __builtin_amdgcn_ballot_w64(mine && (w & kFlagHold) == 0u);
    };
    auto ch_next = [&]() -> uint32_t {
        while (ch_mask == 0ull) {
            const uint64_t nx = (uint64_t)ch_lo + 64ull * gridDim.x;
            if (nx >= (uint64_t)p.channels) return p.channels;
            ch_lo = (uint32_t)nx;
            uint32_t w; bool mine;
            ch_scan(w, mine);
            ch_take(w, mine);
        }
        const uint32_t k = (uint32_t)__builtin_ctzll(ch_mask);
        ch_mask &= ch_mask - 1ull;
        return ch_lo + k * gridDim.x;
    };
    uint32_t w_first; bool mine_first;
    ch_scan(w_first, mine_first);
    uint32_t c = blockIdx.x, c_nx = 0u;
    float *tab = lds + GS::oTab;
    _Float16 *X = reinterpret_cast<_Float16 *>(lds + GS::oX);
    v2f *Hf = reinterpret_cast<v2f *>(lds + GS::oHf);
    float *D = lds + GS::oD;
    float *dI = D, *dQ = D + G::DLEN;
    constexpr int NLD = G::T / 128;
    constexpr int NTL = GS::HS / 128;
    static_assert(GS::HS % 128 == 0 && NTL >= 1 && NTL <= NLD, "history is a whole number of wave loads");

    const uint32_t dec2 = DEC2 ? fa.dec2 : 0u;
    const uint32_t MO = dec2 ? 2u * (uint32_t)M : (uint32_t)M;
    const uint32_t pq = GROUP == 0 ? fa.pass_out : (uint32_t)G::P, tq = pq * MO;
    const uint32_t npass = (p.nout + pq - 1) / pq;
    const uint32_t tail_out = p.nout - (npass - 1) * pq;
    auto cur_out = [&](uint32_t pass) { return pass + 1 == npass ? tail_out : pq; };
    auto in_rsrc = [&](uint32_t ch) {
        return make_rsrc(src + (size_t)ch * p.in_stride * 2, ch < p.channels ? p.block_size * (R::kBytes / 2) : 0u);
    };
    __amdgpu_buffer_rsrc_t rs_in = in_rsrc(c), rs_in_next = in_rsrc(c);
    __amdgpu_buffer_rsrc_t rs_out = make_rsrc(dst + (size_t)c * p.out_stride, p.nout * (W::kBytes / 4));
    const uint32_t env_nblk = ENV ? p.block_size / p.block : 0u;
    auto env_rsrc = [&](uint32_t ch) { return make_rsrc(p.env_part + (size_t)ch * env_nblk, env_nblk * 4u); };
    __amdgpu_buffer_rsrc_t rs_env = env_rsrc(ENV ? c : 0u);
    const __amdgpu_buffer_rsrc_t rs_lo = make_rsrc(p.lo, NCO == 2 ? p.block_size * 8u : 0u);
    const int kInPass = (int)tq * (R::kBytes / 2);

    typename R::type raw[NLD];
    constexpr int LOD = 3;
    u4v lo4[LOD];
    auto lo_load = [&](int slot, int i, int sl) {
        lo4[slot] = __builtin_amdgcn_raw_buffer_load_b128(rs_lo, lane * 16 + i * 1024, sl, 0);
    };
    auto lo_base = [&](uint32_t pass) { return pass < npass ? (int)(pass * tq) * 8 : 0; };
    u4v lo_per[2];
    static_assert((NCO != 3 && NCO != 4) || G::T % 256 == 0, "a pass is a whole number of LO periods");
    if constexpr (NCO == 3) {
        lo_per[0] = *reinterpret_cast<const u4v *>(p.lo + 2 * lane);
        lo_per[1] = *reinterpret_cast<const u4v *>(p.lo + 128 + 2 * lane);
    }
    auto prefetch = [&](uint32_t pass) {
        const int so = pass < npass ? (int)pass * kInPass : 0;
        const __amdgpu_buffer_rsrc_t rs = pass < npass ? rs_in : rs_in_next;
#pragma unroll
        for (int i = 0; i < NLD; ++i) raw[i] = R::load(rs, lane * R::kBytes + i * 64 * R::kBytes, so);
        if constexpr (NCO == 2) {
#pragma unroll
            for (int i = 0; i < LOD; ++i) lo_load(i, i, lo_base(pass));
        }
    };
    prefetch(0);
    h8 Bh[GS::KS], Bl[GS::KS];
    {
        const h8 *bt = static_cast<const h8 *>(fa.btab16);
#pragma unroll
        for (int kk = 0; kk < GS::KS; ++kk) {
            Bh[kk] = bt[(2 * kk + 0) * 64 + lane];
            Bl[kk] = bt[(2 * kk + 1) * 64 + lane];
        }
    }
    float hreg[(NH + 63) / 64];
#pragma unroll
    for (int v = 0; v < (NH + 63) / 64; ++v) hreg[v] = (64 * v + lane < NH) ? p.hilb_c[64 * v + lane] : 0.0f;
    ch_take(w_first, mine_first);
    {
        const uint32_t c_real = ch_next();
        if (c_real >= p.channels) return;
        if (c_real != c) {
            c = c_real;
            rs_in = in_rsrc(c);
            rs_out = make_rsrc(dst + (size_t)c * p.out_stride, p.nout * (W::kBytes / 4));
            if constexpr (ENV != 0) rs_env = env_rsrc(c);
            prefetch(0);
        }
        c_nx = ch_next();
    }
    rs_in_next = in_rsrc(c_nx);

    auto htap = [&](int k) { return __int_as_float(__builtin_amdgcn_readlane(__float_as_int(hreg[k >> 6]), k & 63)); };
    if constexpr (NCO == 1 || NCO == 4)
        for (int i = lane; i < 513; i += kWave) tab[i] = p.sintab[i];

    constexpr int NHI = GS::HS / kWave, NFI = 2 * G::HH4 / kWave;
    static_assert(GS::HS % kWave == 0 && (2 * G::HH4) % kWave == 0, "state fills are whole wave loads");
    v2f st_hv[NHI];
    float st_fv[NFI], st_gain;
    uint32_t st_ph0, st_step, st_word;
    auto load_state = [&](uint32_t ch) {
        const int ndr = (int)p.nd, Fr = G::HQ4 * M + 1 - ndr;
        ch = ch < p.channels ? ch : p.channels - 1;
        const float *stI = p.dec_state + (size_t)ch * 2 * (ndr - 1), *stQ = stI + (ndr - 1);
        const float *stF = p.fir_state + (size_t)ch * 2 * G::HH;
#pragma unroll
        for (int j = 0; j < NHI; ++j) {
            const int s = j * kWave + lane - Fr, sc = s < 0 ? 0 : s;
            const float xi = st_ld(stI + sc), xq = st_ld(stQ + sc);
            st_hv[j] = s < 0 ? v2f{ 0.0f, 0.0f } : v2f{ xi, xq };
        }
#pragma unroll
        for (int j = 0; j < NFI; ++j) {
            const int i = j * kWave + lane;
            const int rail = i / G::HH4, sidx = i % G::HH4 - G::FH;
            const float x = st_ld(stF + rail * G::HH + (sidx < 0 ? 0 : sidx));
            st_fv[j] = sidx < 0 ? 0.0f : x;
        }
        st_ph0 = NCO ? p.phase[ch] : 0u;
        st_step = NCO ? p.step[ch] : 0u;
        st_gain = p.gain[ch];
        st_word = p.rerun_flag ? p.rerun_flag[ch] : 0u;
    };
    uint32_t prev_prov = kProvExact, prev_buf = 0u, st_word_cur = 0u;
    static_assert(ND % 2 == 0 && M * (G::HH4 - G::HH) >= 1, "hist_ext rows are pair-aligned for even tap counts");
    const int ext_start = (int)p.block_size - ((int)p.nd - 1) - (int)p.ext_len + 1;
    const bool ext_on = keeps && p.hist_ext != nullptr && ext_start >= 0;
    __amdgpu_buffer_rsrc_t rs_ext = make_rsrc(p.hist_ext, 0u);
    uint32_t b_hist = 0, ph0 = 0, step = 0;
    float gain = 1.0f;
    int s_cur = 0x7fff;
    float thr_cur = 0.0f, thr_prev = 0.0f, thr_pp = 0.0f;
    uint32_t b_last = 0u;
    GuardPass gd;
    gd.thr = 0.0f; gd.n = 0u; gd.hist = 0ull; gd.nh = 0u; gd.thr_h = 0.0f;
    if constexpr (GROUP == 16) gd.first = 0x0001000100010001ull;
    else if constexpr (GROUP == 32) gd.first = 0x0000000100000001ull;
    else if constexpr (GROUP == 64) gd.first = 1ull;
    else {
        gd.first = 0ull;
        for (int l = 0; l < 64; l += (int)fa.group) gd.first |= 1ull << l;
    }
    const int hist_lanes = ((G::HH + 4 * (int)fa.group - 1) / (4 * (int)fa.group)) * (int)fa.group;
    const uint64_t hist_mask = hist_lanes >= 64 ? ~0ull : ((1ull << hist_lanes) - 1ull);
    gd.hm = AM == 0 ? hist_mask : (fm ? ((GROUP ? GROUP : (int)fa.group) >= 64 ? ~0ull : ((1ull << (GROUP ? GROUP : (int)fa.group)) - 1ull)) : 0ull);
    if constexpr (GROUP != 0 && AM == 0) {
        constexpr int hl = ((G::HH + 4 * GROUP - 1) / (4 * GROUP)) * GROUP;
        gd.hm = hl >= 64 ? ~0ull : ((1ull << hl) - 1ull);
    }
    auto install_state = [&]() {
        float mh = 0.0f;
#pragma unroll
        for (int j = 0; j < NHI; ++j) {
            Hf[j * kWave + lane] = st_hv[j];
            mh = amax2(st_hv[j], mh);
        }
#pragma unroll
        for (int j = 0; j < NFI; ++j) {
            const int i = j * kWave + lane;
            D[(i / G::HH4) * G::DLEN + i % G::HH4] = st_fv[j];
        }
        b_hist = wave_umax_bits(mh);
        ph0 = st_ph0; step = st_step; gain = st_gain;
// ... 235 lines not shown
#pragma unroll
                for (int r = 0; r < 4; ++r) {
                    const float i2 = di[r] + 0.0f;
                    au[r] = fa.upper ? (i2 - q2[r]) : (i2 + q2[r]);
                }
                agc_pass<GROUP>(p.agcp, p.agc, lane, group, au, gain, nvb, gd);
            }
        }
    };
    static_assert(TPK * GS::KS >= NTS, "every Hilbert step has a k-step");
    auto demod = [&](float (&au)[4], int nvb) {
#pragma unroll
        for (int kk = 0; kk < GS::KS; ++kk) demod_piece(kk, au, nvb);
    };
    bool nonfinite = false;
    auto store_audio = [&](uint32_t q, const float (&au)[4]) {
        const float z = __builtin_fmaf(au[3], 0.0f, __builtin_fmaf(au[2], 0.0f, __builtin_fmaf(au[1], 0.0f, au[0] * 0.0f)));
        nonfinite = nonfinite || ((z != z) && (!DEC2 || (uint32_t)lane < pq / 4u));
        const int vo = (GROUP != 0 || (uint32_t)lane < pq / 4u) ? lane * W::kBytes : 0x40000000;
        W::store(rs_out, vo, (int)(q * pq) * (W::kBytes / 4), au, ENV != 0, p.q15_round);
        if constexpr (GROUP == 16 && ENV != 0) {
            {
                const float m = row16_fmax(fmaxf(fmaxf(fabsf(au[0]), fabsf(au[1])), fmaxf(fabsf(au[2]), fabsf(au[3]))));
                const int voff = (lane & 15) == 0 ? (lane >> 4) * 4 : 0x40000000;
                __builtin_amdgcn_raw_buffer_store_b32(__float_as_uint(m), rs_env, voff, (int)q * 16, 0);
            }
        }
    };

    for (;;) {
        install_state();
        float au[4] = { 0.0f, 0.0f, 0.0f, 0.0f };
        lds_order();
        if (DEC2 ? cur_out(0) * MO != (uint32_t)G::T : cur_out(0) != G::P) mix(0, std::true_type{});
        else mix(0, std::false_type{});
        prefetch(1);
        lds_order();
        {
            u4v cb[NCB];
            mfma_phase([](int) {});
            cb_read(cb);
            lds_order();
            cb_write(cb);
            dwrite();
        }
        lds_order();
        for (uint32_t pass = 1; pass < npass; ++pass) {
            if (DEC2 ? cur_out(pass) * MO != (uint32_t)G::T : cur_out(pass) != G::P) mix(pass, std::true_type{});
            else mix(pass, std::false_type{});
            store_audio(pass - 2, au);
            prefetch(pass + 1);
            lds_order();
            u4v cb[NCB];
            v4f dt = { 0.0f, 0.0f, 0.0f, 0.0f };
            if (keeps) dt = *reinterpret_cast<const v4f *>(D + dt_off + pq);
            gd.thr = thr_prev; gd.thr_h = fmaxf(thr_prev, thr_pp);
            gd.hist = pass == 1 ? hist_mask : 0ull;
            const int nvb_full = GROUP == 0 ? (int)(pq / (4u * (uint32_t)group)) : 64;
            mfma_phase([&](int kk) { demod_piece(kk, au, nvb_full); });
            cb_read(cb);
            lds_order();
            cb_write(cb);
            if (keeps) *reinterpret_cast<v4f *>(D + dt_off) = dt;
            dwrite();
            lds_order();
        }
        store_audio(npass - 2, au);
        load_state(c_nx);
        gd.thr = thr_cur; gd.thr_h = fmaxf(thr_cur, thr_prev);
        gd.hist = npass == 1 ? hist_mask : 0ull;
        demod(au, (int)(tail_out / (4u * (uint32_t)group)));
        store_audio(npass - 1, au);

        const bool keep_state = gd.n != 0u && p.rerun_flag != nullptr;
        if (lane == 0) {
            if (gd.n != 0u && p.guard_ch) { p.guard_ch[c] = sat_add_u32(p.guard_ch[c], gd.n); p.guard_calls[c] = sat_add_u32(p.guard_calls[c], 1u); }
            if (keeps && gd.nh != 0u && (prev_prov == kProvSplit || (prev_prov == kProvSplitExt && !p.hist_ext)) && p.guard_hand) p.guard_hand[c] = sat_add_u32(p.guard_hand[c], gd.nh);
            if (p.rerun_flag) {
                const uint32_t kept = !keeps ? (((prev_prov == kProvExact ? kProvExact : kProvSplit) << kProvShift) | (prev_buf << kExtBufShift))
                                              : (((ext_on ? kProvSplitExt : kProvSplit) << kProvShift) | ((prev_buf ^ 1u) << kExtBufShift) |
                                                 (ext_on && sizeof(TIn) == 2 ? kExtQ15 : 0u));
                p.rerun_flag[c] = keep_state ? (kFlagRerun | (st_word_cur & (kExtQ15 | (kProvMask << kProvShift) | (1u << kExtBufShift))))
                                             : (kept | ((b_last + 0xFFu) & kLvlMask));
            }
        }
        lds_order();
        if (!keep_state) {
            const int ndr = (int)p.nd, Fr = G::HQ4 * M + 1 - ndr;
            float *stI = p.dec_state + (size_t)c * 2 * (ndr - 1), *stQ = stI + (ndr - 1);
#pragma unroll
            for (int j = 0; j < GS::HS / kWave; ++j) {
                const int s = j * kWave + lane - Fr;
                const v2f h = Hf[j * kWave + lane];
                if (s >= 0) { st_st(stI + s, h.x); st_st(stQ + s, h.y); }
            }
        }
        if (keeps) {
            int lane_o = lane;
            asm volatile("" : "+v"(lane_o));
            if (!keep_state)
                for (int i = lane_o; i < 2 * G::HH4; i += kWave) {
                    const int rail = i / G::HH4, mi = i % G::HH4, s = mi - G::FH;
                    if (s >= 0) st_st(p.fir_state + ((size_t)c * 2 + rail) * G::HH + s, D[rail * G::DLEN + tail_out + mi]);
                }
        }
        if (lane == 0 && !keep_state) {
            if constexpr (NCO != 0) p.phase[c] = ph0 + p.block_size * step;
            if (p.agc) p.gain[c] = gain;
        }
        c = c_nx;
        if (c >= p.channels) break;
        c_nx = ch_next();
        lds_order();
        rs_in = rs_in_next;
        rs_in_next = in_rsrc(c_nx);
        rs_out = make_rsrc(dst + (size_t)c * p.out_stride, p.nout * (W::kBytes / 4));
        if constexpr (ENV != 0) rs_env = env_rsrc(c);
    }
    if (nonfinite) p.flags[0] = 1u;
}

template <int NCO, int NH, typename TIn, typename TOut, int AM = 0>
__global__ __launch_bounds__(64, 2) void k_hilb_split16(RxParams p, FusedArgs fa, const TIn *__restrict__ src,
                                                        TOut *__restrict__ dst)
{
    using GH = GeoH<NH>;
    using R = BRaw<TIn>;
    using W = BOut<TOut>;
    extern __shared__ __attribute__((aligned(16))) float lds[];
    const int lane = threadIdx.x;
    const uint32_t c = blockIdx.x;
    constexpr bool INLT = AM == 0;
    uint32_t word_t = 0u;
    do {
    if (p.rerun_flag != nullptr) {
        const uint32_t w0 = p.rerun_flag[c];
        if ((w0 & kFlagHold) != 0u) {
            if (INLT && fa.inl != 0u) word_t = w0;
            break;
        }
    }
    float *tab = lds + GH::oTab;
    _Float16 *Xh = reinterpret_cast<_Float16 *>(lds + GH::oX), *Xl = Xh + GH::IMG;
    float *dI = lds + GH::oDI, *dQ = lds + GH::oDQ, *O = lds + GH::oO;
    const uint32_t pq = fa.pass_out;
    const uint32_t npass = (p.nout + pq - 1u) / pq;
    const uint32_t tail_out = p.nout - (npass - 1u) * pq;
    const __amdgpu_buffer_rsrc_t rs_in = make_rsrc(src + (size_t)c * p.in_stride * 2, p.block_size * (R::kBytes / 2));
    const __amdgpu_buffer_rsrc_t rs_out = make_rsrc(dst + (size_t)c * p.out_stride, p.nout * (W::kBytes / 4));
    const __amdgpu_buffer_rsrc_t rs_lo = make_rsrc(p.lo, NCO == 2 ? p.block_size * 8u : 0u);
    const int kInPass = (int)pq * (R::kBytes / 2);
    typename R::type raw[2];
    u4v lo4[2];
    auto prefetch = [&](uint32_t pass) {
        const int so = pass < npass ? (int)pass * kInPass : (int)(p.block_size * (R::kBytes / 2));
#pragma unroll
        for (int i = 0; i < 2; ++i) raw[i] = R::load(rs_in, (uint32_t)(128 * i + 2 * lane) < pq ? lane * R::kBytes + i * 64 * R::kBytes : 0x40000000, so);
        if constexpr (NCO == 2) {
            const int sl = pass < npass ? (int)(pass * pq) * 8 : (int)p.block_size * 8;
#pragma unroll
            for (int i = 0; i < 2; ++i) lo4[i] = __builtin_amdgcn_raw_buffer_load_b128(rs_lo, (uint32_t)(128 * i + 2 * lane) < pq ? lane * 16 + i * 1024 : 0x40000000, sl, 0);
        }
    };
    prefetch(0);

    h8 Bh[GH::KS], Bl[GH::KS];
    {
        const h8 *bt = static_cast<const h8 *>(fa.btab16);
#pragma unroll
        for (int kk = 0; kk < GH::KS; ++kk) {
            Bh[kk] = bt[(2 * kk + 0) * 64 + lane];
            Bl[kk] = bt[(2 * kk + 1) * 64 + lane];
        }
    }
    if constexpr (NCO == 1)
        for (int i = lane; i < 513; i += kWave) tab[i] = p.sintab[i];
    auto put = [&](int u, float x0, float x1, float pre) {
        const v2f s = v2f{ x0, x1 } * v2f{ pre, pre };
        const h2 h = __builtin_convertvector(s, h2);
        const h2 l = __builtin_convertvector(s - __builtin_convertvector(h, v2f), h2);
        const int ph = GH::phys(u);
        *reinterpret_cast<h2 *>(Xh + ph) = h;
        *reinterpret_cast<h2 *>(Xl + ph) = l;
    };
    for (int u = GH::HH + 256 + 2 * lane; u < GH::XN; u += 2 * kWave) put(u, 0.0f, 0.0f, 1.0f);
    const int hv = 2 * lane < GH::HH ? 2 * lane : GH::HH - 2;
    uint32_t b_hist;
    {
        const float *stI = p.fir_state + (size_t)c * 2 * GH::HH, *stQ = stI + GH::HH;
        const float i0 = stI[hv], i1 = stI[hv + 1], q0 = stQ[hv], q1 = stQ[hv + 1];
        *reinterpret_cast<float2 *>(dI + hv) = make_float2(i0, i1);
        *reinterpret_cast<float2 *>(dQ + hv) = make_float2(q0, q1);
        b_hist = wave_umax_bits_dpp(fmaxf(fabsf(q0), fabsf(q1)));
    }
    GuardPass gd{ 0.0f, 1ull, 0u };
    const int group = (int)fa.group;
    if (pq != 256u || group != 64) {
        gd.first = 0ull;
        for (int l = 0; l < 64; l += group) gd.first |= 1ull << l;
    }
    const uint32_t ph0 = NCO ? p.phase[c] : 0u, step = NCO ? p.step[c] : 0u;
    float gain = p.gain[c];
// ... 86 lines not shown
            }
#pragma unroll
            for (int r = 0; r < 4; ++r) {
                const int n = 64 * rg + 16 * r + mcol;
                const float o = i2[r] + q2[r];
                O[n] = o;
                m_mx = fmaxf(m_mx, fabsf(o));
            }
            m_pre = m_mx;
            lds_order();
        }
        {
            const float4 o4 = lds_ld4f(O + 4 * lane);
            au[0] = o4.x; au[1] = o4.y; au[2] = o4.z; au[3] = o4.w;
        }
        if (pq == 256u && group == 64) agc_pass<64>(p.agcp, p.agc, lane, 64, au, gain, 1, gd, m_pre);
        else if (pq == 256u && group == 32) agc_pass<32>(p.agcp, p.agc, lane, 32, au, gain, nvb, gd, m_pre);
        else agc_pass<0>(p.agcp, p.agc, lane, group, au, gain, nvb, gd);
        {
            const float z = __builtin_fmaf(au[3], 0.0f, __builtin_fmaf(au[2], 0.0f, __builtin_fmaf(au[1], 0.0f, au[0] * 0.0f)));
            nonfinite = nonfinite || (z != z);
        }
        W::store(rs_out, (uint32_t)lane < pq / 4u ? lane * W::kBytes : 0x40000000, (int)(pass * pq) * (W::kBytes / 4), au, false, p.q15_round);
        if constexpr (AM == 0) {
            const float2 ti = *reinterpret_cast<const float2 *>(dI + cur + hv);
            const float2 tq = *reinterpret_cast<const float2 *>(dQ + cur + hv);
            const uint32_t th = *reinterpret_cast<const uint32_t *>(Xh + GH::phys((int)cur + hv));
            const uint32_t tl = *reinterpret_cast<const uint32_t *>(Xl + GH::phys((int)cur + hv));
            lds_order();
            *reinterpret_cast<float2 *>(dI + hv) = ti;
            *reinterpret_cast<float2 *>(dQ + hv) = tq;
            *reinterpret_cast<uint32_t *>(Xh + GH::phys(hv)) = th;
            *reinterpret_cast<uint32_t *>(Xl + GH::phys(hv)) = tl;
        }
        lds_order();
    };
    const uint32_t nfull = tail_out == pq ? npass : npass - 1u;
    for (uint32_t pass = 0; pass < nfull; ++pass) one_pass(pass, pq);
    if (nfull != npass) one_pass(nfull, tail_out);
    {
        const bool keep_state = gd.n != 0u && p.rerun_flag != nullptr;
        if (lane == 0) {
            if (gd.n != 0u && p.guard_ch) { p.guard_ch[c] = sat_add_u32(p.guard_ch[c], gd.n); p.guard_calls[c] = sat_add_u32(p.guard_calls[c], 1u); }
            if (p.rerun_flag) p.rerun_flag[c] = keep_state ? 1u : 0u;
        }
        if (keep_state) {
            if (nonfinite) p.flags[0] = 1u;
            if (INLT && fa.inl != 0u) word_t = kFlagRerun;
            break;
        }
    }
    if constexpr (AM == 0) {
        if (2 * lane < GH::HH) {
            float *stI = p.fir_state + (size_t)c * 2 * GH::HH, *stQ = stI + GH::HH;
            const float2 ti = *reinterpret_cast<const float2 *>(dI + hv), tq = *reinterpret_cast<const float2 *>(dQ + hv);
            stI[hv] = ti.x; stI[hv + 1] = ti.y;
            stQ[hv] = tq.x; stQ[hv + 1] = tq.y;
        }
    }
    if (nonfinite) p.flags[0] = 1u;
    if (lane == 0) {
        if constexpr (NCO != 0) p.phase[c] = ph0 + p.block_size * step;
        if (p.agc) p.gain[c] = gain;
    }
    } while (0);
    if constexpr (INLT) {
        if (word_t != 0u) {
            RxParams p2 = p;
            p2.chan_flags = p.rerun_flag;
            p2.rerun_flag = nullptr;
            p2.chan_list = nullptr; p2.chan_count = nullptr; p2.chan_count_next = nullptr; p2.rerun_seen = nullptr;
            FusedArgs fa2 = fa;
            fa2.nco = p.nco == 2 ? 2u : (p.nco == 1 ? ((p.lo_period == 256 && fa.pass_out == 256) ? 4u : 1u) : 0u);
            __syncthreads();
            ssb_fused_body<0, 0, 1, NH, TIn, TOut, 0, true>(p2, fa2, src, dst, FusedInl{ c, word_t });
        }
    }
}

template <int NCO, int ND, int M, int NH, typename TIn, typename TOut, int AM, int GROUP, int FLAVOUR = 0>
static hipError_t launch_k(const RxParams &p, const FusedArgs &fa, const void *src, void *dst, hipStream_t st)
{
    using GS = GeoS<NCO, ND, M, NH>;
    constexpr size_t lds = (size_t)GS::total * sizeof(float);
    static_assert(lds <= 48 * 1024, "k_ssb_split16 LDS image");
    if (fa.inl) return hipErrorNotSupported;
    static int resident = 0;
    if (resident == 0) {
        int per_cu = 0, dev = 0;
        hipDeviceProp_t prop;
        if (hipOccupancyMaxActiveBlocksPerMultiprocessor(&per_cu, k_ssb_split16<NCO, ND, M, NH, TIn, TOut, AM, GROUP, FLAVOUR>, 64, lds) != hipSuccess ||
            hipGetDevice(&dev) != hipSuccess || hipGetDeviceProperties(&prop, dev) != hipSuccess || per_cu <= 0)
            resident = -1;
        else
            resident = per_cu * prop.multiProcessorCount;
        if (const char *e = diag_env("SELENITE_RX_SPLIT16_GRID")) resident = std::atoi(e) > 0 ? std::atoi(e) : -1;
    }
    const uint32_t grid = resident > 0 && (uint32_t)resident < p.channels ? (uint32_t)resident : p.channels;
    if constexpr (GROUP == 16 && AM == 0 && sizeof(TOut) == 4) {
        if (p.env_part) {
            hipLaunchKernelGGL((k_ssb_split16<NCO, ND, M, NH, TIn, TOut, AM, GROUP, 1>), dim3(grid), dim3(64), lds, st, p, fa,
                               static_cast<const TIn *>(src), static_cast<TOut *>(dst));
            return hipGetLastError();
        }
    }
    if (p.env_part) return hipErrorNotSupported;
    hipLaunchKernelGGL((k_ssb_split16<NCO, ND, M, NH, TIn, TOut, AM, GROUP, FLAVOUR>), dim3(grid), dim3(64), lds, st, p, fa,
                       static_cast<const TIn *>(src), static_cast<TOut *>(dst));
    return hipGetLastError();
}

template <int NCO, int ND, int M, int NH, typename TIn, typename TOut>
static hipError_t launch_io(const RxParams &p, const FusedArgs &fa, const void *src, void *dst, hipStream_t st)
{
    if constexpr (M == 4) {
        if (fa.am && fa.dec2) return launch_k<NCO, ND, M, NH, TIn, TOut, 1, 0, 2>(p, fa, src, dst, st);
    }
    if (fa.am && !fa.dec2) return launch_k<NCO, ND, M, NH, TIn, TOut, 1, 0>(p, fa, src, dst, st);
    if constexpr (M == 4) {
        if (fa.dec2) return launch_k<NCO, ND, M, NH, TIn, TOut, 0, 0, 2>(p, fa, src, dst, st);
    }
    if (fa.dec2) return hipErrorNotSupported;
    if constexpr (NCO != 0 && M == 2) {
        if (fa.group == 32) return launch_k<NCO, ND, M, NH, TIn, TOut, 0, 32>(p, fa, src, dst, st);
    } else if constexpr (NCO != 0) {
        if (fa.group == 16) return launch_k<NCO, ND, M, NH, TIn, TOut, 0, 16>(p, fa, src, dst, st);
        if (fa.group == 64) return launch_k<NCO, ND, M, NH, TIn, TOut, 0, 64>(p, fa, src, dst, st);
    }
    return launch_k<NCO, ND, M, NH, TIn, TOut, 0, 0>(p, fa, src, dst, st);
}

template <int ND, int M, int NH, typename T>
static hipError_t launch_nco(const RxParams &p, const FusedArgs &fa, const void *src, void *dst, hipStream_t st)
{
    if constexpr (Geo<ND, M, NH>::T % 256 == 0) {
        if (p.nco == 2 && p.lo_period == 256) return launch_io<3, ND, M, NH, T, T>(p, fa, src, dst, st);
        if (p.nco == 1 && p.lo_period == 256) return launch_io<4, ND, M, NH, T, T>(p, fa, src, dst, st);
    }
    if (p.nco == 2) return launch_io<2, ND, M, NH, T, T>(p, fa, src, dst, st);
    if (p.nco == 1) return launch_io<1, ND, M, NH, T, T>(p, fa, src, dst, st);
    return launch_io<0, ND, M, NH, T, T>(p, fa, src, dst, st);
}

hipError_t launch_ssb_split16_q15(int nd, int m, int nh, const RxParams &p, const FusedArgs &fa, const void *src, void *dst, hipStream_t st);

}
```

### selenite-lite_amd/selenite_rx/__init__.py

```python
import ctypes as C
import os
import subprocess

import numpy as np

_HERE = os.path.dirname(os.path.abspath(__file__))
PKG_ROOT = os.path.dirname(_HERE)
LIB_PATH = os.path.join(PKG_ROOT, "libselenite_rx.so")
if os.environ.get("SELENITE_RX_LIB"):
    LIB_PATH = os.environ["SELENITE_RX_LIB"]

MODE_LSB, MODE_USB, MODE_CW, MODE_CWR, MODE_AM, MODE_FM, MODE_DIG, MODE_PKT = 0, 1, 2, 3, 4, 8, 0x0A, 0x0C
ARITH_CMSIS, ARITH_FMA, ARITH_SPLIT16, ARITH_AUTO = 0, 1, 2, 3
ABI_VERSION, CONFIG_SIZE_V1, TX_CONFIG_SIZE_V1 = 2, 112, 96
OPT_FORCE_GENERIC, OPT_NO_SHARED_LO, OPT_NO_PERIODIC_LO, OPT_RERUN_GRID, OPT_TX_FORCE_GENERIC, OPT_CW_GRID = 0, 1, 2, 3, 4, 5
SUCCESS, ARGUMENT_ERROR, LENGTH_ERROR, NANINF, DEVICE_ERROR = 0, -1, -2, -4, -7
NR_OFF, NR_DENOISE, NR_NOTCH = 0, 1, 2
OUT_MONO, OUT_STEREO = 0, 1
WINDOW_HANN, WINDOW_BLACKMAN_HARRIS = 0, 1

f32p = C.POINTER(C.c_float)
u32p = C.POINTER(C.c_uint32)
i16p = C.POINTER(C.c_int16)
u64p = C.POINTER(C.c_uint64)


class Config(C.Structure):
    _fields_ = [
        ("struct_size", C.c_uint32), ("channels", C.c_uint32), ("block", C.c_uint32),
        ("decim", C.c_uint32), ("nd_taps", C.c_uint32), ("nh_taps", C.c_uint32),
        ("n_biquad", C.c_uint32), ("arith", C.c_uint32),
        ("mode", C.c_uint8), ("nco_enable", C.c_uint8), ("agc_enable", C.c_uint8), ("agc_global", C.c_uint8),
        ("nco_step_all", C.c_uint32),
        ("dec_coeffs", f32p), ("hilb_coeffs", f32p), ("delay_coeffs", f32p), ("biquad_coeffs", f32p),
        ("nco_step", u32p),
        ("agc_target", C.c_float), ("agc_attack", C.c_float), ("agc_decay", C.c_float),
        ("agc_gain_min", C.c_float), ("agc_gain_max", C.c_float), ("agc_env_floor", C.c_float),
        ("agc_gain_init", C.c_float),
        ("q15_rounding", C.c_uint32), ("abi_version", C.c_uint32), ("reserved", C.c_uint32),
    ]


class StateView(C.Structure):
    _fields_ = [("dec_state", f32p), ("fir_state", f32p), ("biq_state", f32p),
                ("agc_gain", f32p), ("nco_phase", u32p)]


class NrConfig(C.Structure):
    _fields_ = [("struct_size", C.c_uint32), ("kind", C.c_uint32), ("num_taps", C.c_uint32), ("delay", C.c_uint32),
                ("mu", C.c_float), ("coeffs_init", f32p)]


class NrStateView(C.Structure):
    _fields_ = [("coeffs", f32p), ("window", f32p), ("delay", f32p), ("energy", f32p), ("x0", f32p)]


class OutConfig(C.Structure):
    _fields_ = [("struct_size", C.c_uint32), ("interp", C.c_uint32), ("ni_taps", C.c_uint32), ("frames", C.c_uint32),
                ("coeffs", f32p)]


class SpecConfig(C.Structure):
    _fields_ = [("struct_size", C.c_uint32), ("fft_len", C.c_uint32), ("stride", C.c_uint32), ("average", C.c_uint32),
                ("alpha", C.c_float), ("window", f32p)]


class SpecStateView(C.Structure):
    _fields_ = [("rows", f32p), ("pending", f32p), ("position", u64p)]


ABI_SYMBOLS = [
    "selenite_rx_init", "selenite_rx_free", "selenite_rx_set_mode", "selenite_rx_status",
    "selenite_rx_error_string", "selenite_rx_process_f32", "selenite_rx_process_f32_device",
    "selenite_rx_process_q15", "selenite_rx_process_q15_device",
    "selenite_rx_global_phase1_device", "selenite_rx_global_phase2_device",
    "selenite_rx_set_stream", "selenite_rx_sync", "selenite_rx_get_state", "selenite_rx_set_state",
    "selenite_rx_reset", "selenite_rx_device_alloc", "selenite_rx_device_free",
    "selenite_rx_memcpy_h2d", "selenite_rx_memcpy_d2h", "selenite_rx_device_count",
    "selenite_rx_set_device", "selenite_rx_synth_iq_host", "selenite_rx_synth_iq_device",
    "selenite_rx_time_process_device", "selenite_rx_time_process_q15_device", "selenite_rx_kernel_name", "selenite_rx_nco_path", "selenite_rx_algorithmic_bytes",
    "selenite_rx_design_lowpass", "selenite_rx_design_hilbert", "selenite_rx_design_bandpass",
    "selenite_rx_abi_version",
    "selenite_rx_global_process_f32_device",
    "selenite_rx_host_alloc", "selenite_rx_host_free", "selenite_rx_host_register", "selenite_rx_host_unregister",
    "selenite_rx_time_process_each_device", "selenite_rx_time_streaming_roof_device", "selenite_rx_time_pattern_roof_device", "selenite_rx_device_pci_bus_id", "selenite_rx_set_plan_option", "selenite_rx_get_plan_option",
    "selenite_rx_set_guard_ratio", "selenite_rx_guard_stats", "selenite_rx_guard_channels", "selenite_rx_auto_words", "selenite_rx_guard_handover", "selenite_rx_set_handover_repair", "selenite_rx_set_auto_launches", "selenite_rx_auto_launches_last", "selenite_rx_guard_clear",
    "selenite_rx_set_nr", "selenite_rx_get_nr_state", "selenite_rx_set_nr_state",
    "selenite_rx_set_out", "selenite_rx_out_values", "selenite_rx_get_out_state", "selenite_rx_set_out_state", "selenite_rx_design_interp",
    "selenite_rx_set_spectrum", "selenite_rx_get_spectrum", "selenite_rx_spectrum_device", "selenite_rx_get_spectrum_state",
    "selenite_rx_set_spectrum_state", "selenite_rx_spectrum_twiddles", "selenite_rx_design_window",
]

class TxConfig(C.Structure):
    _fields_ = [
        ("struct_size", C.c_uint32), ("channels", C.c_uint32), ("block", C.c_uint32),
        ("interp", C.c_uint32), ("ni_taps", C.c_uint32), ("nh_taps", C.c_uint32),
        ("arith", C.c_uint8), ("mode", C.c_uint8), ("nco_enable", C.c_uint8), ("alc_enable", C.c_uint8),
        ("nco_step_all", C.c_uint32),
        ("interp_coeffs", f32p), ("hilb_coeffs", f32p), ("delay_coeffs", f32p), ("nco_step", u32p),
        ("alc_target", C.c_float), ("alc_attack", C.c_float), ("alc_decay", C.c_float),
        ("alc_gain_min", C.c_float), ("alc_gain_max", C.c_float), ("alc_env_floor", C.c_float),
        ("alc_gain_init", C.c_float),
        ("q15_rounding", C.c_uint32), ("abi_version", C.c_uint32), ("reserved", C.c_uint32),
    ]


class TxStateView(C.Structure):
    _fields_ = [("fir_state", f32p), ("interp_state", f32p), ("alc_gain", f32p), ("nco_phase", u32p)]


TX_ABI_SYMBOLS = [
    "selenite_tx_init", "selenite_tx_free", "selenite_tx_set_mode", "selenite_tx_status", "selenite_tx_error_string",
    "selenite_tx_kernel_name",
    "selenite_tx_process_f32", "selenite_tx_process_q15", "selenite_tx_process_f32_device",
    "selenite_tx_process_q15_device", "selenite_tx_set_stream", "selenite_tx_sync", "selenite_tx_get_state",
    "selenite_tx_set_state", "selenite_tx_reset", "selenite_tx_time_process_device",
]

RING_ABI_SYMBOLS = [
    "selenite_ring_init", "selenite_ring_free", "selenite_ring_status", "selenite_ring_error_string",
    "selenite_ring_set_stream", "selenite_ring_sync",
    "selenite_ring_in_write_device", "selenite_ring_in_read_device",
    "selenite_ring_out_write_device", "selenite_ring_out_read_device", "selenite_ring_mute",
    "selenite_ring_in_write", "selenite_ring_in_read", "selenite_ring_out_write", "selenite_ring_out_read",
    "selenite_ring_get_state", "selenite_ring_set_state", "selenite_ring_time_device",
]

_lib = None


def build(force=False):
    if force:
        subprocess.run(["make", "-s", "-C", PKG_ROOT, "clean"], check=True)
    subprocess.run(["make", "-s", "-j4", "-C", PKG_ROOT], check=True)


def lib():
    global _lib
    if _lib is None:
        if not os.path.exists(LIB_PATH):
            raise RuntimeError(
                "libselenite_rx.so is not built (run __graft_entry__.build() or make -C selenite-lite_amd); "
                "there is no CPU fallback for the RX chain")
        L = C.CDLL(LIB_PATH)
        vp = C.c_void_p
        L.selenite_rx_init.argtypes = [C.POINTER(vp), C.POINTER(Config)]
        L.selenite_rx_free.argtypes = [vp]
        L.selenite_rx_set_mode.argtypes = [vp, C.c_uint8]
        L.selenite_rx_status.argtypes = [vp]
        L.selenite_rx_error_string.argtypes = [vp]
        L.selenite_rx_error_string.restype = C.c_char_p
        L.selenite_rx_process_f32.argtypes = [vp, f32p, f32p, C.c_uint32]
        L.selenite_rx_process_f32_device.argtypes = [vp, vp, vp, C.c_uint32]
        L.selenite_rx_process_q15.argtypes = [vp, i16p, i16p, C.c_uint32]
        L.selenite_rx_process_q15_device.argtypes = [vp, vp, vp, C.c_uint32]
        L.selenite_rx_global_phase1_device.argtypes = [vp, vp, vp, vp, C.c_uint32]
        L.selenite_rx_global_phase2_device.argtypes = [vp, vp, vp, C.c_uint32]
        L.selenite_rx_set_stream.argtypes = [vp, vp]
        L.selenite_rx_sync.argtypes = [vp]
        L.selenite_rx_get_state.argtypes = [vp, C.POINTER(StateView)]
        L.selenite_rx_set_state.argtypes = [vp, C.POINTER(StateView)]
        L.selenite_rx_reset.argtypes = [vp]
        L.selenite_rx_device_alloc.argtypes = [C.c_size_t]
        L.selenite_rx_device_alloc.restype = vp
        L.selenite_rx_device_free.argtypes = [vp]
        L.selenite_rx_host_alloc.argtypes = [C.c_size_t]
        L.selenite_rx_host_alloc.restype = vp
        L.selenite_rx_host_free.argtypes = [vp]
        L.selenite_rx_host_free.restype = None
        L.selenite_rx_host_register.argtypes = [vp, C.c_size_t]
        L.selenite_rx_host_unregister.argtypes = [vp]
        L.selenite_rx_memcpy_h2d.argtypes = [vp, vp, C.c_size_t]
        L.selenite_rx_memcpy_d2h.argtypes = [vp, vp, C.c_size_t]
        L.selenite_rx_set_device.argtypes = [C.c_int]
        L.selenite_rx_synth_iq_host.argtypes = [f32p, C.c_uint32, C.c_uint32, C.c_uint64, C.c_uint32, C.c_uint64]
        L.selenite_rx_synth_iq_device.argtypes = [vp, vp, C.c_uint32, C.c_uint32, C.c_uint64, C.c_uint32, C.c_uint64]
        L.selenite_rx_time_process_device.argtypes = [vp, vp, vp, C.c_uint32, C.c_uint32, f32p]
        L.selenite_rx_kernel_name.argtypes = [vp]
        L.selenite_rx_kernel_name.restype = C.c_char_p
        L.selenite_rx_nco_path.argtypes = [vp]
        L.selenite_rx_nco_path.restype = C.c_char_p
        L.selenite_rx_algorithmic_bytes.argtypes = [C.POINTER(Config), C.c_uint32, C.POINTER(C.c_uint64)]
        L.selenite_rx_algorithmic_bytes.restype = C.c_uint64
        u64p = C.POINTER(C.c_uint64)
        L.selenite_rx_time_process_each_device.argtypes = [vp, vp, vp, C.c_uint32, C.c_uint32, f32p, C.c_int]
        L.selenite_rx_time_streaming_roof_device.argtypes = [vp, vp, vp, C.c_uint32, C.c_uint32, f32p, C.c_int]
        if hasattr(L, "selenite_rx_set_plan_option"):
            L.selenite_rx_set_plan_option.argtypes = [C.c_int, C.c_uint32]
            L.selenite_rx_get_plan_option.argtypes = [C.c_int]
            L.selenite_rx_get_plan_option.restype = C.c_uint32
            L.selenite_rx_time_pattern_roof_device.argtypes = [vp, vp, vp, C.c_uint32, C.c_uint32, f32p, C.c_int, C.c_uint32]
        L.selenite_rx_device_pci_bus_id.argtypes = [C.c_int, C.c_char_p, C.c_size_t]
        L.selenite_rx_set_guard_ratio.argtypes = [vp, C.c_float]
        L.selenite_rx_guard_stats.argtypes = [vp, u64p, u64p, u64p]
        L.selenite_rx_guard_channels.argtypes = [vp, u32p]
        L.selenite_rx_auto_words.argtypes = [vp, u32p]
        L.selenite_rx_guard_clear.argtypes = [vp]
        L.selenite_rx_guard_handover.argtypes = [vp, u64p]
        L.selenite_rx_set_handover_repair.argtypes = [vp, C.c_int]
        L.selenite_rx_set_auto_launches.argtypes = [vp, C.c_int]
        L.selenite_rx_auto_launches_last.argtypes = [vp]
        if hasattr(L, "selenite_rx_set_nr"):
            L.selenite_rx_set_nr.argtypes = [vp, C.POINTER(NrConfig)]
            L.selenite_rx_get_nr_state.argtypes = [vp, C.POINTER(NrStateView)]
            L.selenite_rx_set_nr_state.argtypes = [vp, C.POINTER(NrStateView)]
        if hasattr(L, "selenite_rx_set_out"):
            L.selenite_rx_set_out.argtypes = [vp, C.POINTER(OutConfig)]
            L.selenite_rx_out_values.argtypes = [vp, C.c_uint32]
            L.selenite_rx_out_values.restype = C.c_uint32
            L.selenite_rx_get_out_state.argtypes = [vp, f32p]
            L.selenite_rx_set_out_state.argtypes = [vp, f32p]
            L.selenite_rx_design_interp.argtypes = [f32p, C.c_uint32, C.c_uint32, C.c_double]
        if hasattr(L, "selenite_rx_set_spectrum"):
            L.selenite_rx_set_spectrum.argtypes = [vp, C.POINTER(SpecConfig)]
            L.selenite_rx_get_spectrum.argtypes = [vp, f32p, u64p]
            L.selenite_rx_spectrum_device.argtypes = [vp]
            L.selenite_rx_spectrum_device.restype = vp
            L.selenite_rx_get_spectrum_state.argtypes = [vp, C.POINTER(SpecStateView)]
            L.selenite_rx_set_spectrum_state.argtypes = [vp, C.POINTER(SpecStateView)]
            L.selenite_rx_spectrum_twiddles.argtypes = [f32p, C.c_uint32]
            L.selenite_rx_design_window.argtypes = [f32p, C.c_uint32, C.c_int]
        L.selenite_rx_design_lowpass.argtypes = [f32p, C.c_uint32, C.c_double]
        L.selenite_rx_design_hilbert.argtypes = [f32p, f32p, C.c_uint32]
        L.selenite_rx_design_bandpass.argtypes = [f32p, C.c_uint32, C.c_double, C.c_double]
        _lib = L
    return _lib


def _fp(a):
    return a.ctypes.data_as(f32p)


def device_pci_bus_id(ordinal):
    buf = C.create_string_buffer(32)
    rc = lib().selenite_rx_device_pci_bus_id(ordinal, buf, 32)
    return buf.value.decode() if rc == 0 else "unknown"


def design_lowpass(num_taps, cutoff):
    h = np.empty(num_taps, np.float32)
    rc = lib().selenite_rx_design_lowpass(_fp(h), num_taps, cutoff)
    if rc:
        raise ValueError("selenite_rx_design_lowpass: %d" % rc)
    return h


def design_interp(ni_taps, interp, cutoff):
    h = np.empty(ni_taps, np.float32)
    rc = lib().selenite_rx_design_interp(_fp(h), ni_taps, interp, cutoff)
    if rc:
        raise ValueError("selenite_rx_design_interp: %d" % rc)
    return h


def design_window(n, kind=WINDOW_HANN):
    w = np.empty(n, np.float32)
    rc = lib().selenite_rx_design_window(_fp(w), n, kind)
    if rc:
        raise ValueError("selenite_rx_design_window: %d" % rc)
    return w


def spectrum_twiddles(fft_len):
    tw = np.empty((fft_len, 2), np.float32)
    rc = lib().selenite_rx_spectrum_twiddles(_fp(tw), fft_len)
    if rc:
        raise ValueError("selenite_rx_spectrum_twiddles: %d" % rc)
    return tw


def design_hilbert(num_taps):
    h, d = np.empty(num_taps, np.float32), np.empty(num_taps, np.float32)
    rc = lib().selenite_rx_design_hilbert(_fp(h), _fp(d), num_taps)
    if rc:
        raise ValueError("selenite_rx_design_hilbert: %d" % rc)
    return h, d


def design_bandpass(n_stages, f0, q):
    c = np.empty(5 * n_stages, np.float32)
    rc = lib().selenite_rx_design_bandpass(_fp(c), n_stages, f0, q)
    if rc:
        raise ValueError("selenite_rx_design_bandpass: %d" % rc)
    return c
# ... 102 lines not shown
    def process(self, iq, out=None):
        iq = np.ascontiguousarray(iq, np.float32)
        c, bs = iq.shape[0], iq.shape[1]
        if out is None:
            out = np.empty((c, self.out_len(bs)), np.float32)
        self.L.selenite_rx_process_f32(self.h, _fp(iq), _fp(out), bs)
        self.check()
        return out

    def process_q15(self, iq, out=None):
        iq = np.ascontiguousarray(iq, np.int16)
        c, bs = iq.shape[0], iq.shape[1]
        if out is None:
            out = np.empty((c, self.out_len(bs)), np.int16)
        self.L.selenite_rx_process_q15(self.h, iq.ctypes.data_as(i16p), out.ctypes.data_as(i16p), bs)
        self.check()
        return out

    def process_device(self, d_src, d_dst, block_size):
        self.L.selenite_rx_process_f32_device(self.h, d_src, d_dst, block_size)

    def process_q15_device(self, d_src, d_dst, block_size):
        self.L.selenite_rx_process_q15_device(self.h, d_src, d_dst, block_size)

    def global_phase1(self, d_src, d_dst, d_env, block_size):
        self.L.selenite_rx_global_phase1_device(self.h, d_src, d_dst, d_env, block_size)

    def global_phase2(self, d_dst, d_env, block_size):
        self.L.selenite_rx_global_phase2_device(self.h, d_dst, d_env, block_size)

    def set_mode(self, mode):
        return self.L.selenite_rx_set_mode(self.h, mode)

    def set_stream(self, stream_ptr):
        return self.L.selenite_rx_set_stream(self.h, stream_ptr)

    def sync(self):
        rc = self.L.selenite_rx_sync(self.h)
        if rc:
            raise RxError(rc, self.error())

    def reset(self):
        return self.L.selenite_rx_reset(self.h)

    def status(self):
        return self.L.selenite_rx_status(self.h)

    def error(self):
        return self.L.selenite_rx_error_string(self.h).decode()

    def check(self):
        rc = self.status()
        if rc:
            raise RxError(rc, self.error())

    def kernel_name(self):
        return self.L.selenite_rx_kernel_name(self.h).decode()

    def set_guard_ratio(self, ratio):
        rc = self.L.selenite_rx_set_guard_ratio(self.h, ratio)
        if rc:
            raise RxError(rc, "selenite_rx_set_guard_ratio")

    def guard_stats(self):
        b, c, r = C.c_uint64(), C.c_uint64(), C.c_uint64()
        rc = self.L.selenite_rx_guard_stats(self.h, C.byref(b), C.byref(c), C.byref(r))
        if rc:
            raise RxError(rc, self.error())
        h = C.c_uint64()
        rc = self.L.selenite_rx_guard_handover(self.h, C.byref(h))
        if rc:
            raise RxError(rc, self.error())
        return dict(blocks=int(b.value), channel_calls=int(c.value), rerun_channel_calls=int(r.value), handover_blocks=int(h.value))

    def set_handover_repair(self, on):
        return self.L.selenite_rx_set_handover_repair(self.h, int(bool(on)))

    def set_auto_launches(self, launches):
        return self.L.selenite_rx_set_auto_launches(self.h, int(launches))

    def auto_launches_last(self):
        return int(self.L.selenite_rx_auto_launches_last(self.h))

    def guard_channels(self):
        out = np.zeros(self.cfg.channels, np.uint32)
        rc = self.L.selenite_rx_guard_channels(self.h, out.ctypes.data_as(u32p))
        if rc:
            raise RxError(rc, self.error())
        return out

    def auto_words(self):
        out = np.zeros(self.cfg.channels, np.uint32)
        rc = self.L.selenite_rx_auto_words(self.h, out.ctypes.data_as(u32p))
        if rc:
            raise RxError(rc, self.error())
        return out

    def guard_clear(self):
        return self.L.selenite_rx_guard_clear(self.h)

    def nco_path(self):
        return self.L.selenite_rx_nco_path(self.h).decode()

    def time_process(self, d_src, d_dst, block_size, iters):
        ms = C.c_float()
        rc = self.L.selenite_rx_time_process_device(self.h, d_src, d_dst, block_size, iters, C.byref(ms))
        if rc:
            raise RxError(rc, self.error())
        return ms.value

    def time_process_q15(self, d_src, d_dst, block_size, iters):
        ms = C.c_float()
        self.L.selenite_rx_time_process_q15_device.argtypes = [C.c_void_p, C.c_void_p, C.c_void_p, C.c_uint32,
                                                               C.c_uint32, C.POINTER(C.c_float)]
        rc = self.L.selenite_rx_time_process_q15_device(self.h, d_src, d_dst, block_size, iters, C.byref(ms))
        if rc:
            raise RxError(rc, self.error())
        return ms.value

    def time_process_each(self, d_src, d_dst, block_size, iters, q15=False):
        ms = np.zeros(iters, np.float32)
        rc = self.L.selenite_rx_time_process_each_device(self.h, d_src, d_dst, block_size, iters, _fp(ms), int(q15))
        if rc:
            raise RxError(rc, self.error())
        return ms

    def time_streaming_roof(self, d_src, d_dst, block_size, iters, q15=False):
        ms = np.zeros(iters, np.float32)
        rc = self.L.selenite_rx_time_streaming_roof_device(self.h, d_src, d_dst, block_size, iters, _fp(ms), int(q15))
        if rc:
            raise RxError(rc, self.error())
        return ms

    def time_pattern_roof(self, d_src, d_dst, block_size, iters, q15=False, work=0):
        ms = np.zeros(iters, np.float32)
        rc = self.L.selenite_rx_time_pattern_roof_device(self.h, d_src, d_dst, block_size, iters, _fp(ms), int(q15), int(work))
        if rc:
            raise RxError(rc, self.error())
        return ms

    def synth_device(self, d_iq, first_channel, nch, first_sample, nsamp, seed):
        rc = self.L.selenite_rx_synth_iq_device(self.h, d_iq, first_channel, nch, first_sample, nsamp, seed)
        if rc:
            raise RxError(rc, self.error())

    def algorithmic_bytes(self, block_size):
        rd = C.c_uint64()
        tot = self.L.selenite_rx_algorithmic_bytes(C.byref(self.cfg), block_size, C.byref(rd))
        return int(tot), int(rd.value)

    def _state_arrays(self):
        g = self.cfg
        c = g.channels
        return dict(
            dec_state=np.zeros((c, 2, max(g.nd_taps - 1, 0)), np.float32),
            fir_state=np.zeros((c, 2, max(g.nh_taps - 1, 0)), np.float32),
            biq_state=np.zeros((c, g.n_biquad, 4), np.float32),
            agc_gain=np.zeros((c,), np.float32),
            nco_phase=np.zeros((c,), np.uint32),
        )

    @staticmethod
    def _view(arrs):
        v = StateView()
        v.dec_state = _fp(arrs["dec_state"]) if arrs["dec_state"].size else None
        v.fir_state = _fp(arrs["fir_state"]) if arrs["fir_state"].size else None
# ... 404 lines not shown
```

Before: 476,600.

## Fold hist-exact repair into rerun kernel via per-workgroup rerun lists

In the auto-arithmetic split16 SSB path, each split16 workgroup now records the channels it flags for rerun in a strided per-workgroup list and publishes a count. The exact rerun kernel prefix-scans these counts to find its channels, and it runs the history-exact repair inline instead of as a separate launch. The goal is to cut the rerun path from three launches to two and to remove the compaction and repair launches. In exchange, the kernels gain extra LDS bookkeeping and scan logic, and a new knob lets callers pin the grid size.

```diff
diff --git a/include/selenite_rx.h b/include/selenite_rx.h
--- a/include/selenite_rx.h
+++ b/include/selenite_rx.h
@@ -165,6 +165,8 @@
 int selenite_rx_set_handover_repair(selenite_rx_instance *S, int on);
 int selenite_rx_set_auto_launches(selenite_rx_instance *S, int launches);
 int selenite_rx_auto_launches_last(const selenite_rx_instance *S);
+int selenite_rx_auto_launch_count_last(const selenite_rx_instance *S);
+int selenite_rx_set_split16_grid(selenite_rx_instance *S, uint32_t workgroups);
 int selenite_rx_guard_handover(selenite_rx_instance *S, uint64_t *handover_blocks);
 int selenite_rx_guard_clear(selenite_rx_instance *S);
 
diff --git a/selenite-lite_amd/csrc/rx_api.hip b/selenite-lite_amd/csrc/rx_api.hip
--- a/selenite-lite_amd/csrc/rx_api.hip
+++ b/selenite-lite_amd/csrc/rx_api.hip
@@ -99,7 +99,7 @@
 
 static void free_device(selenite_rx_instance *S)
 {
-    void *ptrs[] = { S->d_flags, S->d_guard_ch, S->d_rerun_flag, S->d_rerun_list, S->d_hist_ext, S->d_conv_in, S->d_dec_c, S->d_hilb_c, S->d_delay_c, S->d_biq_c, S->d_sintab, S->d_step, S->d_phase,
+    void *ptrs[] = { S->d_flags, S->d_guard_ch, S->d_rerun_flag, S->d_rerun_list, S->d_wg_sum, S->d_hist_ext, S->d_conv_in, S->d_dec_c, S->d_hilb_c, S->d_delay_c, S->d_biq_c, S->d_sintab, S->d_step, S->d_phase,
                      S->d_dec_state, S->d_fir_state, S->d_biq_state, S->d_gain, S->d_scratch, S->d_env, S->d_env_part,
                      S->d_io_in, S->d_io_out, S->d_lo, S->pipe.d_in[0], S->pipe.d_in[1], S->pipe.d_out[0], S->pipe.d_out[1],
                      S->d_nr_coeffs, S->d_nr_window, S->d_nr_delay, S->d_nr_energy, S->d_nr_x0,
@@ -317,6 +317,7 @@
     INITCHK(dev_alloc(&S->d_guard_ch, 3 * C));
     INITCHK(dev_alloc(&S->d_rerun_flag, cfg->arith == SELENITE_ARITH_AUTO ? C : 0));
     INITCHK(dev_alloc(&S->d_rerun_list, cfg->arith == SELENITE_ARITH_AUTO ? C + 2 : 0));
+    INITCHK(dev_alloc(&S->d_wg_sum, cfg->arith == SELENITE_ARITH_AUTO ? C + 4 : 0));
     if (cfg->arith == SELENITE_ARITH_AUTO) {
         INITCHK(hipHostMalloc(reinterpret_cast<void **>(&S->h_rerun_seen), sizeof(uint32_t), hipHostMallocMapped));
         *S->h_rerun_seen = 0u;
@@ -492,7 +493,19 @@
 
 extern "C" int selenite_rx_auto_launches_last(const selenite_rx_instance *S)
 {
-    return S ? (int)S->auto_form_last : 0;
+    return S ? (int)(S->auto_form_last & 0xFFu) : 0;
+}
+
+extern "C" int selenite_rx_set_split16_grid(selenite_rx_instance *S, uint32_t workgroups)
+{
+    if (!S || workgroups > (1u << 20)) return SELENITE_RX_ARGUMENT_ERROR;
+    S->split16_grid = workgroups;
+    return SELENITE_RX_SUCCESS;
+}
+
+extern "C" int selenite_rx_auto_launch_count_last(const selenite_rx_instance *S)
+{
+    return S ? (int)(S->auto_form_last >> 8) : 0;
 }
 
 extern "C" int selenite_rx_set_handover_repair(selenite_rx_instance *S, int on)
@@ -918,6 +931,7 @@
     bool env_emitted = false;
     if (ssb_fused || cw_fused) {
         RxParams pf = p;
+        pf.grid_pin = S->split16_grid;
         if (g.nco_enable && S->steps_uniform && S->phase_uniform && !S->no_shared_lo) {
             const uint32_t lo_n = block_size < 256u ? 256u : block_size;
             if (!(S->lo_valid && S->lo_phase == phase_now && S->lo_step == S->h_step[0] && S->lo_n >= lo_n)) {
@@ -940,6 +954,7 @@
             pf.rerun_par_host = &S->rerun_par;
             pf.rerun_seen = S->h_rerun_seen;
             pf.auto_inline = S->auto_launches == 1 ? 1u : 0u;
+            pf.wg_sum = S->d_wg_sum;
             pf.form_host = &S->auto_form_last;
         }
         void *fdst = dst;
diff --git a/selenite-lite_amd/csrc/rx_fused.hip b/selenite-lite_amd/csrc/rx_fused.hip
--- a/selenite-lite_amd/csrc/rx_fused.hip
+++ b/selenite-lite_amd/csrc/rx_fused.hip
@@ -446,6 +446,7 @@
         RxParams p2 = p;
         p2.chan_flags = p.rerun_flag;
         p2.rerun_flag = nullptr;
+        p2.wg_sum = nullptr;
         if (p.rerun_par_host) {
             const uint32_t par = *p.rerun_par_host & 1u;
             p2.chan_count = p.chan_count + par;
@@ -479,8 +480,23 @@
                 p3.chan_list = nullptr; p3.chan_count_next = nullptr;
                 if (hipError_t e = launch_hist_exact(p3, true, st); e != hipSuccess) return e;
             }
-            if (auto_ && p.rerun_flag && p.form_host) *p.form_host = 3u;
-            hipError_t e = launch_ssb_split16(nds, M == 8 ? 4 : M, NH, p, fa16, src, src_q15, dst, st);
+            const bool two = auto_ && p.rerun_flag && p.auto_inline && p.wg_sum && p.chan_list;
+            uint32_t mgrid = 0u;
+            RxParams pm = p;
+            if (!two) pm.wg_sum = nullptr;
+            pm.wg_grid_host = &mgrid;
+            if (auto_ && p.rerun_flag && p.form_host) *p.form_host = 3u | ((two ? 2u : 3u) << 8);
+            hipError_t e = launch_ssb_split16(nds, M == 8 ? 4 : M, NH, pm, fa16, src, src_q15, dst, st);
+            if (e == hipSuccess && two) {
+                if (mgrid == 0u) return hipErrorUnknown;
+                RxParams p2 = p;
+                p2.chan_flags = p.rerun_flag;
+                p2.rerun_flag = nullptr;
+                p2.chan_count = nullptr; p2.chan_count_next = nullptr;
+                p2.wg_sum_n = mgrid;
+                p2.wg_repair = hist_exact_repairs(p2) ? 1u : 0u;
+                return launch_exact(ND, M, NH, src_q15, p2, fa, src, dst, st);
+            }
             if (e == hipSuccess && auto_ && p.rerun_flag) e = rerun();
             return e;
         }
@@ -491,7 +507,7 @@
             FusedArgs fah = fa;
             const bool inl = auto_ && p.rerun_flag && p.auto_inline && !fa.am;
             fah.inl = inl ? 1u : 0u;
-            if (auto_ && p.rerun_flag && p.form_host) *p.form_host = inl ? 1u : 3u;
+            if (auto_ && p.rerun_flag && p.form_host) *p.form_host = inl ? (1u | (1u << 8)) : (3u | (3u << 8));
             hipError_t e = launch_hilb_split16(NH, p, fah, src, src_q15, dst, st);
             if (e == hipSuccess && auto_ && p.rerun_flag && !inl) e = rerun();
             return e;
diff --git a/selenite-lite_amd/csrc/rx_fused_kernels.h b/selenite-lite_amd/csrc/rx_fused_kernels.h
--- a/selenite-lite_amd/csrc/rx_fused_kernels.h
+++ b/selenite-lite_amd/csrc/rx_fused_kernels.h
@@ -255,8 +255,66 @@
     float *dI = D, *dQ = D + G::DLEN;
     constexpr int NLD = G::T / 128;
     bool nonfinite = false;
+    constexpr bool TAIL = ARITH == 0 && ND > 0 && NH > 0 && DENSE == 0 && !INL;
+    const bool tail = TAIL && p.chan_flags != nullptr && p.wg_sum != nullptr;
     uint32_t li = INL ? 0u : blockIdx.x;
-    const uint32_t ln = INL ? 1u : (p.chan_flags ? *p.chan_count : 0u);
+    uint32_t ln = INL ? 1u : ((p.chan_flags && !tail) ? *p.chan_count : 0u);
+    uint32_t t_own = 0u, t_incl = 0u;
+    const uint32_t ng = TAIL ? p.wg_sum_n : 0u, nq = (ng + 3u) / 4u;
+    auto wave_scan = [&](uint32_t v) {
+#pragma unroll
+        for (int off = 1; off < 64; off <<= 1) {
+            const uint32_t u = (uint32_t)__shfl_up((int)v, off, 64);
+            if (lane >= off) v += u;
+        }
+        return v;
+    };
+    if constexpr (TAIL) {
+        if (tail) {
+            for (uint32_t q0 = 0u; q0 < nq; q0 += 8u * kWave) {
+                u4v v[8];
+#pragma unroll
+                for (int i = 0; i < 8; ++i) {
+                    const uint32_t q = q0 + (uint32_t)lane + 64u * i;
+                    v[i] = *reinterpret_cast<const u4v *>(p.wg_sum + 4u * (q < nq ? q : nq - 1u));
+                }
+#pragma unroll
+                for (int i = 0; i < 8; ++i) {
+                    const uint32_t w0 = 4u * (q0 + (uint32_t)lane + 64u * i);
+                    t_own += (w0 < ng ? v[i].x : 0u) + (w0 + 1u < ng ? v[i].y : 0u) + (w0 + 2u < ng ? v[i].z : 0u) + (w0 + 3u < ng ? v[i].w : 0u);
+                }
+            }
+            t_incl = wave_scan(t_own);
+            ln = (uint32_t)__builtin_amdgcn_readlane((int)t_incl, 63);
+        }
+    }
+    auto list_at = [&](uint32_t e) -> uint32_t {
+        if constexpr (TAIL) {
+            if (tail) {
+                const uint64_t gt = __builtin_amdgcn_ballot_w64(t_incl > e);
+                if (gt == 0ull) return p.channels;
+                const int L = __builtin_ctzll(gt);
+                uint32_t r = e - ((uint32_t)__shfl((int)t_incl, L, 64) - (uint32_t)__shfl((int)t_own, L, 64));
+                for (uint32_t qb = (uint32_t)L; qb < nq; qb += 16u * kWave) {
+                    const uint32_t wi = 4u * (qb + 64u * ((uint32_t)lane >> 2)) + ((uint32_t)lane & 3u);
+                    const uint32_t v = wi < ng ? p.wg_sum[wi] : 0u;
+                    const uint32_t inc = wave_scan(v);
+                    const uint64_t g2 = __builtin_amdgcn_ballot_w64(inc > r);
+                    if (g2 != 0ull) {
+                        const int m = __builtin_ctzll(g2);
+                        const uint32_t j = (uint32_t)__shfl((int)wi, m, 64);
+                        r -= (uint32_t)__shfl((int)inc, m, 64) - (uint32_t)__shfl((int)v, m, 64);
+                        const uint64_t slot = (uint64_t)j + (uint64_t)r * ng;
+                        const uint32_t ch = slot < (uint64_t)p.channels ? p.chan_list[slot] : p.channels;
+                        return ch < p.channels ? ch : p.channels;
+                    }
+                    r -= (uint32_t)__builtin_amdgcn_readlane((int)inc, 63);
+                }
+                return p.channels;
+            }
+        }
+        return p.chan_list[e];
+    };
     if (!INL && p.chan_flags && p.rerun_seen && blockIdx.x == 0 && lane == 0) __hip_atomic_store(p.rerun_seen, ln, __ATOMIC_RELAXED, __HIP_MEMORY_SCOPE_SYSTEM);
     if (p.chan_flags && li >= ln) return;
     if (NCO == 1u || NCO == 4u)
@@ -276,7 +334,10 @@
     }
     auto in_rsrc = [&](uint32_t ch, bool valid) { return make_rsrc(src + (size_t)ch * p.in_stride * 2, valid ? p.block_size * (R::kBytes / 2) : 0u); };
     uint32_t c_cur = INL ? inl.c : blockIdx.x;
-    if (!INL && p.chan_flags) c_cur = li < ln ? p.chan_list[li] : 0u;
+    if (!INL && p.chan_flags) {
+        c_cur = li < ln ? list_at(li) : 0u;
+        if (c_cur >= p.channels) return;
+    }
     typename R::type raw[NLD];
     {
         const __amdgpu_buffer_rsrc_t rs0 = in_rsrc(c_cur, !p.chan_flags || li < ln);
@@ -291,7 +352,8 @@
         if (li >= ln) break;
         li += INL ? 1u : gridDim.x;
         has_nxt = li < ln;
-        c_nxt = has_nxt ? p.chan_list[li] : 0u;
+        c_nxt = has_nxt ? (INL ? 0u : list_at(li)) : 0u;
+        if (c_nxt >= p.channels) { has_nxt = false; ln = li; c_nxt = 0u; }
     }
 
     const size_t out_base = (size_t)c * p.out_stride;
@@ -299,6 +361,15 @@
     const bool rerun_pass = p.chan_flags != nullptr;
     const uint32_t word_in = INL ? inl.word : (rerun_pass ? p.chan_flags[c] : 0u);
     const bool held_in = (word_in & kFlagHold) != 0u;
+    if constexpr (TAIL) {
+        static_assert(2 * (M * G::HH4 + ND - 1) <= M * G::PSF, "hist_exact_channel's scratch fits the decimator image");
+        if (tail && p.wg_repair != 0u && (word_in & kFlagRerun) != 0u && ((word_in >> kProvShift) & kProvMask) == kProvSplitExt) {
+            hist_exact_channel(p, c, word_in, S, lane);
+            if (lane == 0) p.chan_flags[c] = word_in & ~(kProvMask << kProvShift);
+            __threadfence();
+            __syncthreads();
+        }
+    }
     GuardEx gx{ 0.0f, 0.0f, 0u, 0u };
     float hmax = 0.0f;
     const __amdgpu_buffer_rsrc_t rs_in = in_rsrc(c, true);
diff --git a/selenite-lite_amd/csrc/rx_generic.hip b/selenite-lite_amd/csrc/rx_generic.hip
--- a/selenite-lite_amd/csrc/rx_generic.hip
+++ b/selenite-lite_amd/csrc/rx_generic.hip
@@ -508,11 +508,16 @@
     }
 }
 
+bool hist_exact_repairs(const RxParams &p)
+{
+    static const bool off = diag_env("SELENITE_RX_NO_HIST_EXACT") != nullptr;
+    return p.hist_ext && p.nd >= 2 && p.nh >= 2 && !off;
+}
+
 hipError_t launch_hist_exact(const RxParams &p, bool all, hipStream_t st)
 {
     if (!p.chan_flags) return hipSuccess;
-    static const bool off = diag_env("SELENITE_RX_NO_HIST_EXACT") != nullptr;
-    const bool repair = p.hist_ext && p.nd >= 2 && p.nh >= 2 && !off;
+    const bool repair = hist_exact_repairs(p);
     if (!repair && !p.chan_list) return hipSuccess;
     const uint32_t nwin = (p.channels + 63u) / 64u;
     const size_t lds = repair ? 2 * (size_t)(p.ext_len + p.nd - 1u) * sizeof(float) : 0;
diff --git a/selenite-lite_amd/csrc/rx_internal.h b/selenite-lite_amd/csrc/rx_internal.h
--- a/selenite-lite_amd/csrc/rx_internal.h
+++ b/selenite-lite_amd/csrc/rx_internal.h
@@ -53,6 +53,11 @@
     uint32_t *rerun_par_host;
     uint32_t auto_inline;
     uint32_t *form_host;
+    uint32_t *wg_sum;
+    uint32_t wg_sum_n;
+    uint32_t wg_repair;
+    uint32_t *wg_grid_host;
+    uint32_t grid_pin;
     uint32_t *rerun_seen;
     AgcParams agcp;
 };
@@ -75,6 +80,7 @@
 size_t front_generic_lds_bytes(const RxParams &p);
 hipError_t launch_q15_to_f32(const int16_t *src, float *dst, size_t n, hipStream_t st);
 hipError_t launch_hist_exact(const RxParams &p, bool all, hipStream_t st);
+bool hist_exact_repairs(const RxParams &p);
 hipError_t launch_biquad_generic(const RxParams &p, int arith, float *audio, hipStream_t st);
 hipError_t launch_agc_generic(const RxParams &p, int arith, const float *audio, void *dst,
                               bool dst_q15, hipStream_t st);
@@ -202,6 +208,8 @@
     uint32_t *d_rerun_list = nullptr;
     uint32_t rerun_par = 0;
     uint32_t *h_rerun_seen = nullptr;
+    uint32_t split16_grid = 0;
+    uint32_t *d_wg_sum = nullptr;
     int auto_launches = 1;
     uint32_t auto_form_last = 0;
     float2 *d_hist_ext = nullptr;
diff --git a/selenite-lite_amd/csrc/rx_split16_kernels.h b/selenite-lite_amd/csrc/rx_split16_kernels.h
--- a/selenite-lite_amd/csrc/rx_split16_kernels.h
+++ b/selenite-lite_amd/csrc/rx_split16_kernels.h
@@ -149,8 +149,21 @@
         mine = ci < (uint64_t)p.channels;
         w = p.rerun_flag != nullptr ? p.rerun_flag[mine ? ci : 0] : 0u;
     };
+    uint32_t *wg_n = reinterpret_cast<uint32_t *>(lds + GeoS<NCO, ND, M, NH>::total);
     auto ch_take = [&](uint32_t w, bool mine) {
         ch_mask = __builtin_amdgcn_ballot_w64(mine && (w & kFlagHold) == 0u);
+        const uint64_t held = __builtin_amdgcn_ballot_w64(mine && (w & kFlagHold) != 0u);
+        if (held != 0ull && p.wg_sum != nullptr) {
+            const uint32_t n0 = *wg_n;
+            const uint32_t rank = __builtin_amdgcn_mbcnt_hi((uint32_t)(held >> 32), __builtin_amdgcn_mbcnt_lo((uint32_t)held, 0u));
+            if (mine && (w & kFlagHold) != 0u) p.chan_list[blockIdx.x + (n0 + rank) * gridDim.x] = ch_lo + (uint32_t)lane * gridDim.x;
+            lds_order();
+            if (lane == 0) *wg_n = n0 + (uint32_t)__builtin_popcountll(held);
+            lds_order();
+        }
+    };
+    auto wg_leave = [&]() {
+        if (p.wg_sum != nullptr && lane == 0) p.wg_sum[blockIdx.x] = *wg_n;
     };
     auto ch_next = [&]() -> uint32_t {
         while (ch_mask == 0ull) {
@@ -230,10 +243,12 @@
     float hreg[(NH + 63) / 64];
 #pragma unroll
     for (int v = 0; v < (NH + 63) / 64; ++v) hreg[v] = (64 * v + lane < NH) ? p.hilb_c[64 * v + lane] : 0.0f;
+    if (lane == 0) *wg_n = 0u;
+    lds_order();
     ch_take(w_first, mine_first);
     {
         const uint32_t c_real = ch_next();
-        if (c_real >= p.channels) return;
+        if (c_real >= p.channels) { wg_leave(); return; }
         if (c_real != c) {
             c = c_real;
             rs_in = in_rsrc(c);
@@ -635,6 +650,11 @@
                                                  (ext_on && sizeof(TIn) == 2 ? kExtQ15 : 0u));
                 p.rerun_flag[c] = keep_state ? (kFlagRerun | (st_word_cur & (kExtQ15 | (kProvMask << kProvShift) | (1u << kExtBufShift))))
                                              : (kept | ((b_last + 0xFFu) & kLvlMask));
+                if (keep_state && p.wg_sum != nullptr) {
+                    const uint32_t n0 = *wg_n;
+                    p.chan_list[blockIdx.x + n0 * gridDim.x] = c;
+                    *wg_n = n0 + 1u;
+                }
             }
         }
         lds_order();
@@ -671,6 +691,7 @@
         if constexpr (ENV != 0) rs_env = env_rsrc(c);
     }
     if (nonfinite) p.flags[0] = 1u;
+    wg_leave();
 }
 
 template <int NCO, int NH, typename TIn, typename TOut, int AM = 0>
@@ -923,7 +944,7 @@
 static hipError_t launch_k(const RxParams &p, const FusedArgs &fa, const void *src, void *dst, hipStream_t st)
 {
     using GS = GeoS<NCO, ND, M, NH>;
-    constexpr size_t lds = (size_t)GS::total * sizeof(float);
+    constexpr size_t lds = ((size_t)GS::total + 4) * sizeof(float);
     static_assert(lds <= 48 * 1024, "k_ssb_split16 LDS image");
     if (fa.inl) return hipErrorNotSupported;
     static int resident = 0;
@@ -937,7 +958,9 @@
             resident = per_cu * prop.multiProcessorCount;
         if (const char *e = diag_env("SELENITE_RX_SPLIT16_GRID")) resident = std::atoi(e) > 0 ? std::atoi(e) : -1;
     }
-    const uint32_t grid = resident > 0 && (uint32_t)resident < p.channels ? (uint32_t)resident : p.channels;
+    uint32_t grid = resident > 0 && (uint32_t)resident < p.channels ? (uint32_t)resident : p.channels;
+    if (p.grid_pin) grid = p.grid_pin < p.channels ? p.grid_pin : p.channels;
+    if (p.wg_grid_host) *p.wg_grid_host = grid;
     if constexpr (GROUP == 16 && AM == 0 && sizeof(TOut) == 4) {
         if (p.env_part) {
             hipLaunchKernelGGL((k_ssb_split16<NCO, ND, M, NH, TIn, TOut, AM, GROUP, 1>), dim3(grid), dim3(64), lds, st, p, fa,
diff --git a/selenite-lite_amd/selenite_rx/__init__.py b/selenite-lite_amd/selenite_rx/__init__.py
--- a/selenite-lite_amd/selenite_rx/__init__.py
+++ b/selenite-lite_amd/selenite_rx/__init__.py
@@ -84,7 +84,7 @@
     "selenite_rx_global_process_f32_device",
     "selenite_rx_host_alloc", "selenite_rx_host_free", "selenite_rx_host_register", "selenite_rx_host_unregister",
     "selenite_rx_time_process_each_device", "selenite_rx_time_streaming_roof_device", "selenite_rx_time_pattern_roof_device", "selenite_rx_device_pci_bus_id", "selenite_rx_set_plan_option", "selenite_rx_get_plan_option",
-    "selenite_rx_set_guard_ratio", "selenite_rx_guard_stats", "selenite_rx_guard_channels", "selenite_rx_auto_words", "selenite_rx_guard_handover", "selenite_rx_set_handover_repair", "selenite_rx_set_auto_launches", "selenite_rx_auto_launches_last", "selenite_rx_guard_clear",
+    "selenite_rx_set_guard_ratio", "selenite_rx_guard_stats", "selenite_rx_guard_channels", "selenite_rx_auto_words", "selenite_rx_guard_handover", "selenite_rx_set_handover_repair", "selenite_rx_set_auto_launches", "selenite_rx_auto_launches_last", "selenite_rx_auto_launch_count_last", "selenite_rx_set_split16_grid", "selenite_rx_guard_clear",
     "selenite_rx_set_nr", "selenite_rx_get_nr_state", "selenite_rx_set_nr_state",
     "selenite_rx_set_out", "selenite_rx_out_values", "selenite_rx_get_out_state", "selenite_rx_set_out_state", "selenite_rx_design_interp",
     "selenite_rx_set_spectrum", "selenite_rx_get_spectrum", "selenite_rx_spectrum_device", "selenite_rx_get_spectrum_state",
@@ -200,6 +200,9 @@
         L.selenite_rx_set_handover_repair.argtypes = [vp, C.c_int]
         L.selenite_rx_set_auto_launches.argtypes = [vp, C.c_int]
         L.selenite_rx_auto_launches_last.argtypes = [vp]
+        if hasattr(L, "selenite_rx_auto_launch_count_last"):
+            L.selenite_rx_auto_launch_count_last.argtypes = [vp]
+            L.selenite_rx_set_split16_grid.argtypes = [vp, C.c_uint32]
         if hasattr(L, "selenite_rx_set_nr"):
             L.selenite_rx_set_nr.argtypes = [vp, C.POINTER(NrConfig)]
             L.selenite_rx_get_nr_state.argtypes = [vp, C.POINTER(NrStateView)]
@@ -468,6 +471,12 @@
     def auto_launches_last(self):
         return int(self.L.selenite_rx_auto_launches_last(self.h))
 
+    def set_split16_grid(self, workgroups):
+        return self.L.selenite_rx_set_split16_grid(self.h, int(workgroups))
+
+    def auto_launch_count_last(self):
+        return int(self.L.selenite_rx_auto_launch_count_last(self.h))
+
     def guard_channels(self):
         out = np.zeros(self.cfg.channels, np.uint32)
         rc = self.L.selenite_rx_guard_channels(self.h, out.ctypes.data_as(u32p))
```

Measured after the change: 476,100, median of 2. Within noise of the previous version (-0.1%).
